# TurakhiaLab/DIPPER

Hardware: AMD Instinct MI355X
Metric: tips/sec FASTA->Newick at N=30000 (higher is better)
Workload: dtype f64

## Files before the change

### dipper_amd/csrc/njp.hip

```cpp
#include "njp_args.hpp"

#include <algorithm>
#include <chrono>
#include <cstdio>
#include <cstdlib>
#include <functional>
#include <numeric>
#include <string>
#include <type_traits>

namespace dpr {

static int64_t njp_big_p()
{
    static const int64_t v = std::getenv("DPR_NJ_BIG_P") ? std::atoll(std::getenv("DPR_NJ_BIG_P")) : 40000;
    return v;
}
static bool njp_post2_on()
{
    static const bool on = !(std::getenv("DPR_NJP_POST2") && std::atoi(std::getenv("DPR_NJP_POST2")) == 0);
    return on;
}
static int njp_tg(int64_t P) { return P < njp_big_p() ? 64 : 256; }
constexpr int kBigNS = 4;
static int njp_ns(int64_t P) { return P < njp_big_p() ? 1 : kBigNS; }
__host__ __device__ inline int64_t njp_strips_of_rows(int64_t g0, int64_t tg, int64_t P)
{
    const int64_t G16 = (P + 16 - 1) / 16;
    const int64_t glast = (g0 + tg < G16 ? g0 + tg : G16) - 1;
    if (glast < 0) return 0;
    int64_t c = glast / 32 + 1;
    const int64_t cp = (P - 2) / 512 + 1;
    return P >= 2 ? (c < cp ? c : cp) : 0;
}

int njp_unit_owner(int64_t strip, int64_t group, int64_t P, int world)
{
    const int64_t G16 = (P + kUR - 1) / kUR;
    if (strip < 0 || group < 0 || group >= G16 || group < 32 * strip || strip * kTileCols >= P - 1 || world < 1) return -1;
    int64_t t = 0;
    const int64_t tg = njp_tg(P), ns = njp_ns(P);
    if (ns == 1) {
        for (int64_t c = 0; c < strip; ++c) t += (G16 - 32 * c + tg - 1) / tg;
        t += (group - 32 * strip) / tg;
    } else {
        const int64_t k = group / tg;
        for (int64_t kk = 0; kk < k; ++kk) t += (njp_strips_of_rows(kk * tg, tg, P) + ns - 1) / ns;
        t += strip / ns;
    }
    return (int)(t % world);
}

__device__ __forceinline__ void njp_note_range(unsigned long long* mm, double lo, double hi)
{
    if (lo < 0.0) {
        const double cur = dec_f64(mm[0]);
        if (cur >= 0.0 || lo < 2.0 * cur) atomicMin(&mm[0], (unsigned long long)enc_f64(lo));
    }
    if (hi > 0.0) {
        const double cur = dec_f64(mm[1]);
        if (hi > 2.0 * cur) atomicMax(&mm[1], (unsigned long long)enc_f64(hi));
    }
}

__global__ __launch_bounds__(kThreads) void njp_permute_kernel(const double* __restrict__ A, int64_t lda,
                                                               double* __restrict__ B, int64_t ldb,
                                                               const int32_t* __restrict__ perm, int64_t P)
{
    const int xcd = (int)(blockIdx.x & 7u), chunk = (int)(blockIdx.x >> 3), nchunk = (int)(gridDim.x >> 3);
    for (int64_t a = (int64_t)blockIdx.y * 8 + xcd; a < P; a += (int64_t)gridDim.y * 8) {
        const double* row = A + (int64_t)perm[a] * lda;
        for (int64_t b = (int64_t)chunk * kThreads + threadIdx.x; b < P; b += (int64_t)nchunk * kThreads)
            B[a * ldb + b] = row[perm[b]];
    }
}

static void njp_launch_permute(const double* A, int64_t lda, double* B, int64_t ldb, const int32_t* perm, int64_t n, hipStream_t s)
{
    int64_t chunks = (n + 1023) / 1024;
    chunks = chunks < 1 ? 1 : (chunks > 64 ? 64 : chunks);
    const int64_t gy = (n + 7) / 8;
    dim3 grid((unsigned)(8 * chunks), (unsigned)(gy < 32768 ? gy : 32768));
    hipLaunchKernelGGL(njp_permute_kernel, grid, dim3(kThreads), 0, s, A, lda, B, ldb, perm, n);
}

__global__ __launch_bounds__(kThreads) void njp_range_kernel(const double* __restrict__ A, int64_t lda, int64_t n, unsigned long long* __restrict__ mm)
{
    __shared__ double slo[kThreads / 64], shi[kThreads / 64];
    double lo = __builtin_inf(), hi = 0.0;
    for (int64_t a = blockIdx.x; a < n; a += gridDim.x) {
        const double* row = A + a * lda;
        for (int64_t b = threadIdx.x; b < n; b += kThreads) {
            const double v = row[b];
            lo = fmin(lo, v); hi = fmax(hi, fabs(v));
        }
    }
    lo = wave_fmin(lo); hi = wave_fmax(hi);
    if ((threadIdx.x & 63) == 0) { slo[threadIdx.x >> 6] = lo; shi[threadIdx.x >> 6] = hi; }
    __syncthreads();
    if (threadIdx.x == 0) {
        for (int w = 1; w < kThreads / 64; ++w) { lo = fmin(lo, slo[w]); hi = fmax(hi, shi[w]); }
        atomicMin(&mm[0], (unsigned long long)enc_f64(lo));
        atomicMax(&mm[1], (unsigned long long)enc_f64(hi));
    }
}

__global__ __launch_bounds__(kThreads) void njp_init_vectors_kernel(const double* __restrict__ U_src,
                                                                    const int32_t* __restrict__ perm,
                                                                    const int32_t* __restrict__ slot_src,
                                                                    int64_t P, int64_t n, double* __restrict__ U,
                                                                    double* __restrict__ Ur, uint64_t* __restrict__ KA,
                                                                    uint64_t* __restrict__ KB,
                                                                    int32_t* __restrict__ slot_of_pos,
                                                                    int32_t* __restrict__ pos_of_slot)
{
    const int64_t p = (int64_t)blockIdx.x * kThreads + threadIdx.x;
    if (p >= P) return;
    const int32_t src = perm[p];
    const int32_t slot = slot_src ? slot_src[src] : src;
    const double u = U_src[src];
    U[p] = u;
    Ur[p] = u / (double)(n - 2);
    KA[p] = nj_key_a_dev(slot, n);
    KB[p] = nj_key_b(slot);
    slot_of_pos[p] = slot;
    pos_of_slot[slot] = (int32_t)p;
}

__global__ void njp_fill_u64_kernel(uint64_t* __restrict__ a, int64_t cnt, uint64_t v)
{
    for (int64_t i = (int64_t)blockIdx.x * blockDim.x + threadIdx.x; i < cnt; i += (int64_t)gridDim.x * blockDim.x) a[i] = v;
}

__global__ __launch_bounds__(kThreads) void njp_list_all_kernel(NjpArgs a)
{
    const int tid = threadIdx.x;
    const int64_t it = a.st->it;
    if (a.st->status != 0) return;
    const int tb = a.sh_rank + (int)blockIdx.x * a.sh_world;
    const int cb0 = a.blk_cb[tb];
    const int64_t g = (int64_t)a.blk_g0[tb] + tid;
    const int64_t G16 = (a.P + kUR - 1) / kUR;
    const int tg = a.tg;
    int64_t send = njp_strips_of_rows((int64_t)a.blk_g0[tb], tg, a.P);
    if (a.ns == 1) send = cb0 + 1;
    else if (send > cb0 + a.ns) send = cb0 + a.ns;
    const int lane = tid & 63;
    for (int cb = cb0; cb < (int)send; ++cb) {
        const bool keep = g < G16 && g >= 32 * (int64_t)cb && tid < tg;
        const unsigned long long mask = __ballot(keep);
        unsigned long long base = 0;
        if (lane == 0 && mask) base = atomicAdd(&a.cnt[it % 3], (unsigned long long)__popcll(mask));
        base = __shfl(base, 0, 64);
        if (keep) a.list[base + __popcll(mask & ((1ull << lane) - 1ull))] = (int32_t)((0xFu << 28) | ((uint32_t)cb << 18) | (uint32_t)g);
    }
}

template <bool kRS>
__global__ __launch_bounds__(kThreads) void njp_scan_kernel(NjState* h_st, const int32_t* h_list, const unsigned long long* h_cnt,
                                                            const double* h_xpart, int h_nrl, NjpArgs a)
{
    __shared__ double sq[kThreads / 64], sd[kThreads / 64];
    __shared__ uint64_t sk[kThreads / 64], sp[kThreads / 64];
    __shared__ double stree[kThreads];
    __shared__ unsigned int s_last;

    const int tid = threadIdx.x;
    const int64_t it = h_st->it, limit = h_st->it_limit, N = h_st->N;
    const int nrl = h_nrl;
    const bool unit_block = (int)blockIdx.x >= nrl;
    const int ub = (int)blockIdx.x - nrl;
    const int32_t first = unit_block ? h_list[ub] : 0;
    const double xp0 = unit_block ? 0.0 : h_xpart[tid];
    const unsigned long long cl0 = h_cnt[0], cl1 = h_cnt[1], cl2 = h_cnt[2];
    const int64_t j0 = (int64_t)blockIdx.x * kTileCols + 2 * tid;
    v2d dv0, dv1, uv; ulonglong2 kav, kbv;
    dv0.x = dv0.y = 0.0; dv1 = dv0; uv = dv0; kav = make_ulonglong2(0ull, 0ull); kbv = kav;
    if (!unit_block) {
        dv0 = *reinterpret_cast<const v2d*>(a.R + j0);
        dv1 = *reinterpret_cast<const v2d*>(a.R + a.vstride + j0);
        uv = *reinterpret_cast<const v2d*>(a.Ur + j0);
        kav = *reinterpret_cast<const ulonglong2*>(a.KA + j0); kbv = *reinterpret_cast<const ulonglong2*>(a.KB + j0);
    }
    const int32_t pn0 = h_st->pnew[0], pn1 = h_st->pnew[1];
    const int64_t pz = (int64_t)((it & 1) ? pn1 : pn0);
    if (blockIdx.x == 0 && tid == 0) h_st->itb = it;
    if (it >= limit || h_st->status != 0) return;
    NJP_STAMP(0, 0, true);
    const int64_t P = a.P;
    double bq = 10000.0, bd = 0.0;
    uint64_t bk = ~0ull, bp = 0;
    NjRecord* rec_out;

    if (!unit_block) {
        const int r = (int)blockIdx.x;
        rec_out = a.partials + a.urecs + r;
        if (pz < 0) {
            if (tid == 0) { NjRecord rec; rec.q = 10000.0; rec.key = ~0ull; rec.d = 0.0; rec.pad = 0ull; *rec_out = rec; }
            if (kRS) {
                if (r == 0 && tid == 0) njr_store_record(a.partials + a.rec_off - 1, 10000.0, ~0ull, it == a.rs_fault_it ? 1.0e-3 : 0.0, a.rs_seq_base + (unsigned long long)(it + 1));
                njr_scan_publish(a, it, &s_last);
            }
            return;
        }
        const int64_t n = N - it;
        const int64_t nchunk = (n + 1 + kThreads - 1) / kThreads;
        double acc = tid < nchunk ? xp0 : 0.0;
        for (int64_t c = tid + kThreads; c < nchunk; c += kThreads) acc += a.xpart[c];
        const v2d dv = ((it + 1) & 1) ? dv1 : dv0;
        const uint64_t kax = a.KA[pz], kbx = a.KB[pz];
        NJP_STAMP(0, 1, true);
        double ux = block_tree256_lane0(acc, stree);
        if (tid == 0) stree[0] = ux;
        __syncthreads();
        ux = stree[0];
        NJP_STAMP(0, 2, false);
        const double urx = ux / (double)(n - 2);
        if (r == 0 && tid == 0) a.U[(it & 1) * a.vstride + pz] = ux;
        if (kRS && r == 0 && tid == 0)
            njr_store_record(a.partials + a.rec_off - 1, 10000.0, ~0ull, it == a.rs_fault_it ? ux * 0.5 + 1.0e-3 : ux, a.rs_seq_base + (unsigned long long)(it + 1));
        if (j0 < P && njp_owns<kRS>(a, pz)) *reinterpret_cast<v2d*>(a.D + njp_lrow<kRS>(a, pz) * a.ld + j0) = dv;
#pragma unroll
        for (int k = 0; k < 2; ++k) {
            const double d = k ? dv.y : dv.x, uj = k ? uv.y : uv.x;
            const uint64_t kaj = k ? kav.y : kav.x, kbj = k ? kbv.y : kbv.x;
            const uint64_t pj = (uint64_t)(j0 + k);
            best_update4(bq, bk, bp, bd, (d - urx) - uj, kax | kbj, (uint64_t)pz | (pj << 32), d);
            best_update4(bq, bk, bp, bd, (d - uj) - urx, kaj | kbx, pj | ((uint64_t)pz << 32), d);
        }
        wave_best4(bq, bk, bp, bd);
    } else {
        rec_out = a.partials + a.rec_off + ub;
        const int m3 = (int)(it % 3);
        const int64_t cnt = (int64_t)(m3 == 0 ? cl0 : m3 == 1 ? cl1 : cl2);
        if ((int64_t)ub >= cnt) {
            if (a.all_defined && tid == 0) {
                if (kRS) njr_store_record(rec_out, 10000.0, ~0ull, 0.0, 0ull);
                else { NjRecord rec; rec.q = 10000.0; rec.key = ~0ull; rec.d = 0.0; rec.pad = 0ull; *rec_out = rec; }
            }
            if (kRS) njr_scan_publish(a, it, &s_last);
            return;
        }
        const int64_t G16 = (P + kUR - 1) / kUR;
        int64_t scanned = 0;
        const int wv = tid >> 6;
        for (int64_t e = ub; e < cnt; e += a.ugrid, ++scanned) {
            const uint32_t code = (uint32_t)__builtin_amdgcn_readfirstlane(e == (int64_t)ub ? first : a.list[e]);
            if (!((code >> (28 + wv)) & 1u)) continue;
            const int cb = (int)((code >> 18) & 1023u);
            const int64_t g_s = (int64_t)(code & 0x3FFFFu);
            const int64_t c0 = (int64_t)cb * kTileCols, a0 = g_s * kUR;
            const int64_t b0 = c0 + 2 * tid, b1 = b0 + 1;
            const v2d ubv = *reinterpret_cast<const v2d*>(a.Ur + b0);
            const ulonglong2 kav = *reinterpret_cast<const ulonglong2*>(a.KA + b0), kbv = *reinterpret_cast<const ulonglong2*>(a.KB + b0);
            const double ub0 = ubv.x, ub1 = ubv.y;
            const uint64_t ka0 = kav.x, ka1 = kav.y, kb0 = kbv.x, kb1 = kbv.y;
            const v2d* basep = reinterpret_cast<const v2d*>(a.D + njp_lrow<kRS>(a, a0) * a.ld + c0) + tid;
            const int64_t ld2 = a.ld >> 1;
            const bool diag = a0 < c0 + kTileCols;
            const bool live0 = ub0 == ub0, live1 = ub1 == ub1;
            v2d v[kUR];
#pragma unroll
            for (int u8 = 0; u8 < kUR; ++u8) v[u8] = __builtin_nontemporal_load(basep + (int64_t)u8 * ld2);
            const double ua_l = a.Ur[a0 + (tid & 15)];
            const uint64_t kaa_l = a.KA[a0 + (tid & 15)], kba_l = a.KB[a0 + (tid & 15)];
            double ua[kUR];
#pragma unroll
            for (int u8 = 0; u8 < kUR; ++u8) ua[u8] = readlane_f64(ua_l, u8);
            NJP_STAMP(0, 1, true);
            if (diag) {
                const int ib0 = (int)b0, ia0 = (int)a0;
#pragma unroll
                for (int u8 = 0; u8 < kUR; ++u8) {
                    const int ar = ia0 + u8;
                    v[u8].x = (ib0 < ar) ? v[u8].x : __builtin_nan("");
                    v[u8].y = (ib0 + 1 < ar) ? v[u8].y : __builtin_nan("");
                }
            }
            double lm = __builtin_inf(), m0 = __builtin_inf(), m1 = __builtin_inf();
            double rowq[kUR];
#pragma unroll
            for (int u8 = 0; u8 < kUR; ++u8) {
                const double d0 = v[u8].x, d1 = v[u8].y;
                const double rn = ua[u8] == ua[u8] ? 0.0 : __builtin_nan("");
                m0 = fmin(m0, d0 + rn);
                m1 = fmin(m1, d1 + rn);
                const double q0 = (d0 - ua[u8]) - ub0;
                const double q1 = (d0 - ub0) - ua[u8];
                const double q2 = (d1 - ua[u8]) - ub1;
                const double q3 = (d1 - ub1) - ua[u8];
                rowq[u8] = fmin(fmin(q0, q1), fmin(q2, q3));
                lm = fmin(lm, rowq[u8]);
            }
            double m = fmin(fmin(live0 ? m0 : __builtin_nan(""), live1 ? m1 : __builtin_nan("")), __builtin_inf());
            const double wm = wave_fmin(lm);
            NJP_STAMP(0, 2, false);
            if (wm <= bq) {
                if (wm < bq) { bq = wm; bk = ~0ull; }
                if (a.dbg != nullptr && (it == a.dbg_it || a.dbg_it == -2) && (tid & 63) == 0) atomicAdd(&a.dbg[(a.dbg_it == -2 ? 0 : (int)blockIdx.x) * 8 + 6], 1ull);
#pragma unroll
                for (int u8 = 0; u8 < kUR; ++u8) {
                    if (__builtin_amdgcn_ballot_w64(rowq[u8] == wm) != 0ull) {
                        if (a.dbg != nullptr && (it == a.dbg_it || a.dbg_it == -2) && (tid & 63) == 0) atomicAdd(&a.dbg[(a.dbg_it == -2 ? 0 : (int)blockIdx.x) * 8 + 5], 1ull);
                        double d0 = v[u8].x, d1 = v[u8].y;
                        asm volatile("" : "+v"(d0), "+v"(d1));
                        const bool e0 = (d0 - ua[u8]) - ub0 == wm, e1 = (d0 - ub0) - ua[u8] == wm;
                        const bool e2 = (d1 - ua[u8]) - ub1 == wm, e3 = (d1 - ub1) - ua[u8] == wm;
                        const uint64_t pa = (uint64_t)(a0 + u8);
                        const uint64_t kaa = readlane_u64(kaa_l, u8), kba = readlane_u64(kba_l, u8);
                        const uint64_t k0 = kaa | kb0, k1 = ka0 | kba, k2 = kaa | kb1, k3 = ka1 | kba;
                        if (e0 & (k0 < bk)) { bk = k0; bp = pa | ((uint64_t)b0 << 32); bd = d0; }
                        if (e1 & (k1 < bk)) { bk = k1; bp = (uint64_t)b0 | (pa << 32); bd = d0; }
                        if (e2 & (k2 < bk)) { bk = k2; bp = pa | ((uint64_t)b1 << 32); bd = d1; }
                        if (e3 & (k3 < bk)) { bk = k3; bp = (uint64_t)b1 | (pa << 32); bd = d1; }
                    }
                }
            }
            NJP_STAMP(0, 7, false);
            m = wave_fmin(m);
            if ((tid & 63) == 0) a.umin[((int64_t)cb * G16 + g_s) * 4 + wv] = enc_f64(m);
        }
        {
            const uint64_t wk = wave_umin64(bk);
            if (wk != ~0ull) {
                const unsigned long long own = __builtin_amdgcn_ballot_w64(bk == wk);
                const int src = __builtin_amdgcn_readfirstlane((int)__builtin_ctzll(own));
                bp = readlane_u64(bp, src);
                bd = readlane_f64(bd, src);
            }
            bk = wk;
        }
        if (tid == 0) {
            if (ub == 0) atomicAdd(&a.st->units_scanned, (unsigned long long)cnt);
        }
    }
    NJP_STAMP(0, 3, false);
    if ((tid & 63) == 0) { sq[tid >> 6] = bq; sk[tid >> 6] = bk; sp[tid >> 6] = bp; sd[tid >> 6] = bd; }
    __syncthreads();
    if (tid == 0) {
#pragma unroll
        for (int w = 1; w < kThreads / 64; ++w) best_update4(bq, bk, bp, bd, sq[w], sk[w], sp[w], sd[w]);
        if (kRS && unit_block) njr_store_record(rec_out, bq, bk, bd, bp);
        else {
            NjRecord rec;
            rec.q = bq; rec.key = bk; rec.d = bd; rec.pad = bp;
            *rec_out = rec;
        }
    }
    if (kRS) njr_scan_publish(a, it, &s_last);
    NJP_STAMP(0, 4, true);
}

template <bool kRS>
__global__ __launch_bounds__(kThreads) void njp_finish_kernel(NjpArgs a)
{
    __shared__ double stree[kThreads];
    const int tid = threadIdx.x;
    const int64_t it = a.st->it, N = a.st->N;
    const int64_t pz = (int64_t)a.st->pnew[it & 1];
    if (a.st->status != 0 || pz < 0) return;
    const int64_t n = N - it;
    const int64_t nchunk = (n + 1 + kThreads - 1) / kThreads;
    double acc = 0.0;
    for (int64_t c = tid; c < nchunk; c += kThreads) acc += a.xpart[c];
    const double* __restrict__ Rz = a.R + ((it + 1) & 1) * a.vstride;
    const int64_t j0 = (int64_t)blockIdx.x * kTileCols + 2 * tid;
    const v2d dv = *reinterpret_cast<const v2d*>(Rz + j0);
    const double ux = block_tree256_lane0(acc, stree);
    if (blockIdx.x == 0 && tid == 0) a.U[(it & 1) * a.vstride + pz] = ux;
    if (j0 < a.P && njp_owns<kRS>(a, pz)) *reinterpret_cast<v2d*>(a.D + njp_lrow<kRS>(a, pz) * a.ld + j0) = dv;
}

#ifndef DPR_NJP_BIG_WAVES
#define DPR_NJP_BIG_WAVES 1
#endif
template <int kTG, int kNS, bool kRS>
__global__ __launch_bounds__(kThreads, (kNS > 1 ? DPR_NJP_BIG_WAVES : 1)) void njp_post_kernel(NjState* h_st, const NjRecord* h_partials, const unsigned long long* h_cnt, const int32_t* h_blk_cb,
                                                                                              const int32_t* h_blk_g0, const int32_t* h_pos_of_slot, int h_ntest, int h_nupd, NjpArgs a)
{
    __shared__ double s[kThreads];
    __shared__ double sq[kThreads / 64], sdd[kThreads / 64];
    __shared__ uint64_t sk[kThreads / 64], spp[kThreads / 64];
    __shared__ double sseed[kThreads / 64];
    const int tid = threadIdx.x;
    const int bx = (int)blockIdx.x;
    const bool test_block = bx < h_ntest;
    const int tbi = bx, ubi = bx - h_ntest;
    const int tb = test_block ? a.sh_rank + tbi * a.sh_world : 0;
    const int64_t it = h_st->itb;
    const int64_t limit = h_st->it_limit, N = h_st->N;
    const int32_t pn0 = h_st->pnew[0], pn1 = h_st->pnew[1];
    const int64_t pz = (int64_t)((it & 1) ? pn1 : pn0);
    const int nrec_all = a.urecs + a.nrb;
    NjRecord r0; r0.q = 10000.0; r0.key = ~0ull; r0.d = 0; r0.pad = 0;
    constexpr int kMine = 5;
    NjRecord mine[kMine] = { r0, r0, r0, r0, r0 };
#pragma unroll
    for (int k = 0; k < kMine; ++k) {
        const int idx = tid + k * kThreads;
        if (idx < nrec_all) mine[k] = h_partials[idx];
    }
    const int nseed_rows = a.nrb < kThreads / 2 ? a.nrb : kThreads / 2;
    const int nseed_units = kThreads - nseed_rows;
    const int64_t sstride = a.all_defined && a.urecs >= 2 * nseed_units ? a.urecs / nseed_units : 1;
    const bool seed_is_unit = tid < nseed_units;
    NjRecord cand = r0;
    if (test_block) {
        if (!seed_is_unit) cand = h_partials[a.urecs + (tid - nseed_units)];
        else if ((int64_t)tid * sstride < a.urecs) cand = h_partials[(int64_t)tid * sstride];
    }
    const unsigned long long cl0 = h_cnt[0], cl1 = h_cnt[1], cl2 = h_cnt[2];
    const int m3 = (int)(it % 3);
    const unsigned long long cnt_raw = a.all_defined ? (unsigned long long)a.urecs : (m3 == 0 ? cl0 : m3 == 1 ? cl1 : cl2);
    const int64_t uvalid = (int64_t)(cnt_raw < (unsigned long long)a.urecs ? cnt_raw : (unsigned long long)a.urecs);
    const double* __restrict__ Uc = a.U + (it & 1) * a.vstride;
    double* __restrict__ Un = a.U + ((it + 1) & 1) * a.vstride;
    const int64_t P = a.P;
    const int64_t G16 = (P + kUR - 1) / kUR;
    const int64_t pclamp = (P + 1) & ~(int64_t)1;
    const int64_t i = (int64_t)ubi * kThreads + tid;
    int64_t p = -1;
    double up = 0.0;
    struct ColData { v2d ucol, dxc, dyc, rzc; ulonglong2 um0, um1; };
    int cb0 = 0, nsb = 0;
    int64_t g = 0, rbase = 0;
    bool have_g = false;
    constexpr int kRC = kTG * kUR / kTileCols;
    v2d urow[kRC];
    ColData cd[kNS];
#pragma unroll
    for (int k = 0; k < kNS; ++k) {
        cd[k].ucol.x = 0.0; cd[k].ucol.y = 0.0; cd[k].dxc = cd[k].ucol; cd[k].dyc = cd[k].ucol; cd[k].rzc = cd[k].ucol;
        cd[k].um0 = make_ulonglong2(0ull, 0ull); cd[k].um1 = cd[k].um0;
    }
    auto load_a = [&](int cb, ColData& c) {
        const int64_t pc0 = (int64_t)cb * kTileCols + 2 * tid;
        c.ucol = *reinterpret_cast<const v2d*>(Uc + pc0);
        if (have_g && g >= 32 * (int64_t)cb) {
            const unsigned long long* up = a.umin + ((int64_t)cb * G16 + g) * 4;
            c.um0 = *reinterpret_cast<const ulonglong2*>(up); c.um1 = *reinterpret_cast<const ulonglong2*>(up + 2);
        }
    };
    if (test_block) {
        cb0 = h_blk_cb[tb];
        g = (int64_t)h_blk_g0[tb] + tid;
        have_g = g < G16 && tid < kTG;
        rbase = (int64_t)h_blk_g0[tb] * kUR;
        if (kNS == 1) nsb = 1;
        else {
            const int64_t send = njp_strips_of_rows((int64_t)h_blk_g0[tb], kTG, P);
            nsb = (int)(send - cb0 < kNS ? send - cb0 : kNS);
        }
#pragma unroll
        for (int k = 0; k < kNS; ++k)
            if (k < nsb) load_a(cb0 + k, cd[k]);
#pragma unroll
        for (int c = 0; c < kRC; ++c) {
            const int64_t pp = rbase + c * kTileCols + 2 * tid;
            urow[c] = *reinterpret_cast<const v2d*>(Uc + (pp < P ? pp : pclamp));
        }
    } else {
        p = (int64_t)h_pos_of_slot[i];
    }
#pragma unroll
    for (int k = 0; k < kMine; ++k) {
        const int idx = tid + k * kThreads;
        if (idx >= uvalid && idx < a.urecs) mine[k] = r0;
    }
    if (!test_block) up = (i < N && p >= 0) ? Uc[p] : 0.0;
    if (h_st->status != 0 || it >= limit) return;
    const int64_t n = N - it;
    if (n < 3) return;
    if (!test_block && (!a.do_update || (int64_t)ubi * kThreads >= n)) return;
    if (test_block && !a.do_tests) return;
    NJP_STAMP(1, 0, false);
    NJP_STAMP(1, 1, true);

    double bq = 10000.0, d = 0.0; uint64_t bk = ~0ull, bp = 0;
    const int nmine = (nrec_all + kThreads - 1) / kThreads;
#pragma unroll
    for (int k = 0; k < kMine; ++k)
        if (k < nmine) best_update4(bq, bk, bp, d, mine[k].q, mine[k].key, mine[k].pad, mine[k].d);
    for (int64_t idx = tid + kMine * kThreads; idx < nrec_all; idx += kThreads)
        if (idx < uvalid || idx >= a.urecs) best_update4(bq, bk, bp, d, a.partials[idx].q, a.partials[idx].key, a.partials[idx].pad, a.partials[idx].d);
    wave_best4(bq, bk, bp, d);
    if ((tid & 63) == 0) { sq[tid >> 6] = bq; sk[tid >> 6] = bk; spp[tid >> 6] = bp; sdd[tid >> 6] = d; }
    __syncthreads();
    bq = sq[0]; bk = sk[0]; bp = spp[0]; d = sdd[0];
#pragma unroll
    for (int w = 1; w < kThreads / 64; ++w) best_update4(bq, bk, bp, d, sq[w], sk[w], spp[w], sdd[w]);

    NJP_STAMP(1, 2, false);
    const int64_t last = n - 1;
    if (bk == ~0ull || !(bq < 10000.0)) {
        if (!test_block && i == last) a.st->status = 1;
        return;
    }
    const int64_t ki = (int64_t)(bk & 0xFFFFFFull), kj = (int64_t)((bk >> 24) & 0xFFFFFFull);
    const int64_t pi = (int64_t)(bp & 0xffffffffull), pj = (int64_t)(bp >> 32);
    const int64_t x = ki < kj ? ki : kj, y = ki < kj ? kj : ki;
    const int64_t px = ki < kj ? pi : pj, py = ki < kj ? pj : pi;
    const int64_t n1 = n - 1;
    const double r1 = (double)(n1 - 2);
    const double* __restrict__ rowx = kRS ? a.rs_rows : a.D + px * a.ld;
    const double* __restrict__ rowy = kRS ? a.rs_rows + a.rs_slice : a.D + py * a.ld;
    auto RX = [&](int64_t pp_) -> const double* { return kRS ? rowx + njp_xoff(a, pp_) : rowx + pp_; };
    auto RY = [&](int64_t pp_) -> const double* { return kRS ? rowy + njp_xoff(a, pp_) : rowy + pp_; };
    if (kRS && a.rs_plan == kNjrMailbox) {
        __shared__ int s_fail;
        if (tid == 0) s_fail = 0;
        __syncthreads();
        if (tid < a.rs_world) {
            const unsigned long long* f = njr_win_rowflag(a.rs_win[a.rs_rank], a.rs_lay, tid);
            const unsigned long long want = a.rs_seq_base + (unsigned long long)(it + 1), t0 = wall_clock64();
            while (njr_ld_sys(f) != want) {
                if (wall_clock64() - t0 > a.rs_poll_ticks) { s_fail = 1; break; }
                __builtin_amdgcn_s_sleep(1);
            }
        }
        __syncthreads();
        if (s_fail) {
            if (!test_block && i == last) a.st->status = 3;
            return;
        }
    }

    if (!test_block) {
        double* __restrict__ Rw = a.R + (it & 1) * a.vstride;
        double val = 0.0;
        if (i < n) {
            if (i == last) {
                const double r = (double)(n - 2);
                double blX = (d + Uc[px] / r - Uc[py] / r) * 0.5;
                double blY = d - blX;
                if (blX < 0) { blY += blX; blX = 0; }
                if (blY < 0) { blX += blY; blY = 0; }
                a.log_x[it] = (int32_t)x; a.log_y[it] = (int32_t)y; a.log_bx[it] = blX; a.log_by[it] = blY;
                a.st->x = (int32_t)x; a.st->y = (int32_t)y; a.st->d = d; a.st->q = bq;
                a.st->n = n1; a.st->it = it + 1;
                a.st->pnew[(it + 1) & 1] = (int32_t)px;
                a.U[(it & 1) * a.vstride + py] = __builtin_nan("");
                a.st->cnt_list[(it + 2) % 3] = 0ull;
                for (int v = 0; v < a.cnt_ranks; ++v) a.cnt_all[4 * v + (it + 2) % 3] = 0ull;
            }
            int64_t new_slot = i;
            if (i != x && i != y) {
                const double dxi = *RX(p), dyi = *RY(p);
                val = nj_val(dxi, dyi, d);
                const double u = nj_unew(up, dxi, dyi, val);
                Un[p] = u;
                a.Ur[p] = u / r1;
                Rw[p] = val;
                if (kRS) { if (njp_owns<true>(a, p)) __hip_atomic_store(a.D + njp_lrow<true>(a, p) * a.ld + px, val, __ATOMIC_RELAXED, __HIP_MEMORY_SCOPE_AGENT); }
                else __hip_atomic_store(a.D + p * a.ld + px, val, __ATOMIC_RELAXED, __HIP_MEMORY_SCOPE_AGENT);
                if (i == last) {
                    new_slot = y;
                    a.slot_of_pos[p] = (int32_t)y;
                    a.pos_of_slot[y] = (int32_t)p;
                }
            } else if (i == y) {
                a.Ur[py] = __builtin_nan("");
                Un[py] = __builtin_nan("");
                a.slot_of_pos[py] = -1;
                Rw[py] = 0.0;
                new_slot = -1;
            } else {
                a.Ur[px] = __builtin_nan("");
                Rw[px] = 0.0;
            }
            if (new_slot >= 0) { a.KA[p] = nj_key_a_dev(new_slot, n1); a.KB[p] = nj_key_b(new_slot); }
        }
        NJP_STAMP(1, 3, false);
        const double cs = block_tree256_lane0(val, s);
        if (tid == 0) a.xpart[ubi] = cs;
        NJP_STAMP(1, 6, true);
        return;
    }

    const double NINF = -__builtin_inf(), PINF = __builtin_inf();
    const bool fold = pz >= 0 && pz != px && pz != py;
    const double* __restrict__ Rz = a.R + ((it + 1) & 1) * a.vstride;
    const int64_t gz = fold ? pz / kUR : -1;
    const bool gz_here = fold && gz >= (int64_t)a.blk_g0[tb] && gz < (int64_t)a.blk_g0[tb] + kTG;
    const int wpz = fold ? (int)((pz % kTileCols) / (kTileCols / 4)) : -1;
    auto load_b = [&](int cb, ColData& c) {
        const int64_t pc0 = (int64_t)cb * kTileCols + 2 * tid;
        c.dxc = *reinterpret_cast<const v2d*>(RX(pc0));
        c.dyc = *reinterpret_cast<const v2d*>(RY(pc0));
        c.rzc.x = PINF; c.rzc.y = PINF;
        if (gz_here) c.rzc = *reinterpret_cast<const v2d*>(Rz + pc0);
    };
    constexpr bool kPreRz = kRC <= 4;
    const bool pz_block = fold && pz / kTileCols >= cb0 && pz / kTileCols < cb0 + nsb;
    v2d dxr[kRC], dyr[kRC], rzr[kPreRz ? kRC : 1];
#pragma unroll
    for (int c = 0; c < kRC; ++c) {
        const int64_t pp = rbase + c * kTileCols + 2 * tid;
        const int64_t po = pp < P ? pp : pclamp;
        dxr[c] = *reinterpret_cast<const v2d*>(RX(po));
        dyr[c] = *reinterpret_cast<const v2d*>(RY(po));
        if (kPreRz) {
            rzr[c].x = 0.0; rzr[c].y = 0.0;
            if (pz_block) rzr[c] = *reinterpret_cast<const v2d*>(Rz + po);
        }
    }
#pragma unroll
    for (int k = 0; k < kNS; ++k)
        if (k < nsb) load_b(cb0 + k, cd[k]);
    double qc = PINF;
    if (seed_is_unit && (int64_t)tid * sstride >= uvalid) cand.key = ~0ull;
    if (cand.key != ~0ull) {
        const int64_t ci = (int64_t)(cand.pad & 0xffffffffull), cj = (int64_t)(cand.pad >> 32);
        if (ci < P && cj < P && ci != px && cj != px && ci != py && cj != py) {
            const double uia = Uc[ci], uib = Uc[cj];
            const double xa = *RX(ci), ya = *RY(ci), xb = *RX(cj), yb = *RY(cj);
            const double ua = nj_unew(uia, xa, ya, nj_val(xa, ya, d)) / r1;
            const double ub = nj_unew(uib, xb, yb, nj_val(xb, yb, d)) / r1;
            const double qk = fmin((cand.d - ua) - ub, (cand.d - ub) - ua);
            qc = qk == qk ? qk : qc;
        }
    }
    NJP_STAMP(1, 3, true);
    __shared__ double s_un[kTG * (kUR + 1)];
    __shared__ double scm2[2][kThreads / 64], snew2[2][kThreads / 64];
    const int lxp = (int)(px - rbase), lyp = (int)(py - rbase), lzp = (int)((fold ? pz : -1) - rbase);
#pragma unroll
    for (int c = 0; c < kRC; ++c) {
        const int lp = c * kTileCols + 2 * tid;
        const double u0 = urow[c].x, u1 = urow[c].y;
        const bool live0 = (u0 == u0) & (lp != lxp) & (lp != lyp);
        const bool live1 = (u1 == u1) & (lp + 1 != lxp) & (lp + 1 != lyp);
        const double n0 = nj_unew(u0, dxr[c].x, dyr[c].x, nj_val(dxr[c].x, dyr[c].x, d));
        const double n1v = nj_unew(u1, dxr[c].y, dyr[c].y, nj_val(dxr[c].y, dyr[c].y, d));
        const int li = lp + (lp >> 4);
        s_un[li] = live0 ? n0 : NINF;
        s_un[li + 1] = live1 ? n1v : NINF;
    }
    qc = wave_fmin(qc);
    if ((tid & 63) == 0) sseed[tid >> 6] = qc;
    double bound = PINF, rmax = NINF;
    const int tg = tid < kTG ? tid : 0;
    const int lane = tid & 63;
#pragma unroll
    for (int sidx = 0; sidx < kNS; ++sidx) {
        if (sidx >= nsb) break;
        const int cb = cb0 + sidx, par = sidx & 1;
        const ColData& cur = cd[sidx];
        const int64_t pc0 = (int64_t)cb * kTileCols + 2 * tid;
        const bool pz_strip = fold && pz / kTileCols == cb;
        const bool have = have_g && g >= 32 * (int64_t)cb;
        unsigned long long* up4 = a.umin + ((int64_t)cb * G16 + (have ? g : 0)) * 4;
        double u4[4] = { PINF, PINF, PINF, PINF };
        if (have) { u4[0] = dec_f64(cur.um0.x); u4[1] = dec_f64(cur.um0.y); u4[2] = dec_f64(cur.um1.x); u4[3] = dec_f64(cur.um1.y); }
        double cm_part = NINF, colmin = PINF;
#pragma unroll
        for (int k = 0; k < 2; ++k) {
            const int64_t pp = pc0 + k;
            const double uo = k ? cur.ucol.y : cur.ucol.x;
            const double dx = k ? cur.dxc.y : cur.dxc.x, dy = k ? cur.dyc.y : cur.dyc.x;
            const double rz = k ? cur.rzc.y : cur.rzc.x;
            const bool live = (uo == uo) & (pp != px) & (pp != py) & (pp < P);
            const double un = nj_unew(uo, dx, dy, nj_val(dx, dy, d));
            cm_part = live ? fmax(cm_part, un) : cm_part;
            colmin = (live & (pp < pz)) ? fmin(colmin, rz) : colmin;
        }
        cm_part = wave_fmax(cm_part) / r1;
        if (gz_here) colmin = wave_fmin(colmin);
        if (lane == 0) { scm2[par][tid >> 6] = cm_part; snew2[par][tid >> 6] = colmin; }
        __syncthreads();
        NJP_STAMP(1, 4, false);
        if (sidx == 0) {
            bound = fmin(fmin(sseed[0], sseed[1]), fmin(sseed[2], sseed[3]));
#pragma unroll
            for (int k = 0; k < kUR; ++k) rmax = fmax(rmax, s_un[17 * tg + k]);
            rmax = rmax / r1;
        }
        double newminA = PINF;
        if (pz_strip) {
            __syncthreads();
#pragma unroll
            for (int c = 0; c < kRC; ++c) {
                const int lp = c * kTileCols + 2 * tid;
                const int64_t pp = rbase + lp;
                const v2d rz = kPreRz ? rzr[kPreRz ? c : 0] : *reinterpret_cast<const v2d*>(Rz + (pp < P ? pp : pclamp));
                const double u0 = urow[c].x, u1 = urow[c].y;
                const bool live0 = (u0 == u0) & (lp != lxp) & (lp != lyp) & (lp > lzp);
                const bool live1 = (u1 == u1) & (lp + 1 != lxp) & (lp + 1 != lyp) & (lp + 1 > lzp);
                const int li = lp + (lp >> 4);
                s_un[li] = live0 ? rz.x : PINF;
                s_un[li + 1] = live1 ? rz.y : PINF;
            }
            __syncthreads();
#pragma unroll
            for (int k = 0; k < kUR; ++k) newminA = fmin(newminA, s_un[17 * tg + k]);
        }
        int submask = 0;
        if (have) {
#pragma unroll
            for (int w = 0; w < 4; ++w) {
                const double cmw = scm2[par][w];
                double nm = (gz_here && g == gz) ? snew2[par][w] : PINF;
                if (pz_strip && w == wpz) nm = fmin(nm, newminA);
                if (nm < u4[w]) {
                    u4[w] = nm;
                    up4[w] = enc_f64(nm);
                }
                const double lb = fmin((u4[w] - rmax) - cmw, (u4[w] - cmw) - rmax);
                if ((cmw > NINF) && (lb <= bound)) submask |= 1 << w;
            }
        }
        const bool keep = have && (rmax > NINF) && submask != 0;
        const unsigned long long mask = __ballot(keep);
        unsigned long long base = 0;
        if (lane == 0 && mask) base = atomicAdd(&a.cnt[(it + 1) % 3], (unsigned long long)__popcll(mask));
        base = __shfl(base, 0, 64);
        if (a.dbg != nullptr && a.dbg_it == -2 && mask) {
            int subs = keep ? __popc(submask) : 0;
            for (int off = 32; off > 0; off >>= 1) subs += __shfl_xor(subs, off, 64);
            if (lane == 0 && it < 32768) {
                atomicMax(&a.dbg[32768 + it], ((unsigned long long)__popcll(mask) << 32) | (unsigned long long)subs);
                atomicAdd(&a.dbg[7], (unsigned long long)subs);
            }
        }
        NJP_STAMP(1, 5, true);
        if (keep) a.list[base + __popcll(mask & ((1ull << lane) - 1ull))] = (int32_t)(((uint32_t)submask << 28) | ((uint32_t)cb << 18) | (uint32_t)g);
    }
    NJP_STAMP(1, 6, true);
}

struct Post2Hdr { unsigned long long min_enc, maxabs_enc; };

__global__ __launch_bounds__(kThreads) void njp_t2_init_kernel(const double* __restrict__ Uc, int64_t P, double* __restrict__ rmaxU,
                                                               double* __restrict__ cmaxU)
{
    const int tid = threadIdx.x;
    const int64_t p0 = (int64_t)blockIdx.x * kTileCols + 2 * tid;
    const v2d uc = *reinterpret_cast<const v2d*>(Uc + p0);
    const double NINF = -__builtin_inf();
    const double m2 = fmax(((uc.x == uc.x) & (p0 < P)) ? uc.x : NINF, ((uc.y == uc.y) & (p0 + 1 < P)) ? uc.y : NINF);
    double gm = m2;
    gm = fmax(gm, __shfl_xor(gm, 1, 64)); gm = fmax(gm, __shfl_xor(gm, 2, 64)); gm = fmax(gm, __shfl_xor(gm, 4, 64));
    const double cm = wave_fmax(m2);
    if ((tid & 7) == 0) rmaxU[p0 >> 4] = gm;
    if ((tid & 63) == 0) cmaxU[4 * blockIdx.x + (tid >> 6)] = cm;
}

template <int kNS>
__global__ __launch_bounds__(kThreads) void njp_post2_kernel(NjState* h_st, const NjRecord* h_partials, const unsigned long long* h_cnt, const int32_t* h_blk_cb,
                                                         const int32_t* h_blk_g0, const int32_t* h_pos_of_slot, int h_ntest, int h_nupd, NjpArgs a)
{
    constexpr int kTG = 256;
    __shared__ double s[kThreads];
    __shared__ double sq[kThreads / 64], sdd[kThreads / 64];
    __shared__ uint64_t sk[kThreads / 64], spp[kThreads / 64];
    __shared__ double sseed[kThreads / 64], srC[kThreads / 64], scm[kNS * 4], s_colmin[kNS * 4];
    const int tid = threadIdx.x;
    const int lane = tid & 63;
    const int bx = (int)blockIdx.x;
    const bool trole = bx < h_ntest;
    const int tb = a.sh_rank + bx * a.sh_world;
    const int umb = bx - h_ntest;
    Post2Hdr* hdr = reinterpret_cast<Post2Hdr*>(a.t2_hdr);
    const double NINF = -__builtin_inf(), PINF = __builtin_inf();

    const int64_t it = h_st->itb;
    const int64_t limit = h_st->it_limit, N = h_st->N;
    const int32_t pn0 = h_st->pnew[0], pn1 = h_st->pnew[1];
    const int64_t pz = (int64_t)((it & 1) ? pn1 : pn0);
    const int64_t P = a.P;
    const int64_t G16 = (P + kUR - 1) / kUR;
    const int nrec_all = a.urecs + a.nrb;
    NjRecord r0; r0.q = 10000.0; r0.key = ~0ull; r0.d = 0; r0.pad = 0;
    constexpr int kMine = 5;
    NjRecord mine[kMine] = { r0, r0, r0, r0, r0 };
#pragma unroll
    for (int k = 0; k < kMine; ++k) {
        const int idx = tid + k * kThreads;
        if (idx < nrec_all) mine[k] = h_partials[idx];
    }
    const int nseed_rows = a.nrb < kThreads / 2 ? a.nrb : kThreads / 2;
    const int nseed_units = kThreads - nseed_rows;
    const int64_t sstride = a.all_defined && a.urecs >= 2 * nseed_units ? a.urecs / nseed_units : 1;
    const bool seed_is_unit = tid < nseed_units;
    NjRecord cand = r0;
    int cb0 = 0;
    int64_t g0 = 0;
    const int64_t i = (int64_t)umb * (2 * kThreads) + tid;
    const int64_t p0 = (int64_t)umb * kTileCols + 2 * tid;
    const bool m_part = !trole && umb < a.nrb && a.do_update;
    const bool u_slots = !trole && (int64_t)umb * (2 * kThreads) < N;
    int64_t p = -1, pb = -1;
    int2 sl = make_int2(-1, -1);
    if (trole) {
        if (!seed_is_unit) cand = h_partials[a.urecs + (tid - nseed_units)];
        else if ((int64_t)tid * sstride < a.urecs) cand = h_partials[(int64_t)tid * sstride];
        cb0 = h_blk_cb[tb];
        g0 = (int64_t)h_blk_g0[tb];
    } else {
        if (u_slots) { p = (int64_t)h_pos_of_slot[i]; pb = (int64_t)h_pos_of_slot[i + kThreads]; }
        if (m_part) sl = *reinterpret_cast<const int2*>(a.slot_of_pos + p0);
    }
    const int par = (int)(it & 1);
    const double* __restrict__ Uc = a.U + (it & 1) * a.vstride;
    double* __restrict__ Un = a.U + ((it + 1) & 1) * a.vstride;
    const unsigned long long cl0 = h_cnt[0], cl1 = h_cnt[1], cl2 = h_cnt[2];
    const int m3 = (int)(it % 3);
    const unsigned long long cnt_raw = a.all_defined ? (unsigned long long)a.urecs : (m3 == 0 ? cl0 : m3 == 1 ? cl1 : cl2);
    const int64_t uvalid = (int64_t)(cnt_raw < (unsigned long long)a.urecs ? cnt_raw : (unsigned long long)a.urecs);
    const double emin = dec_f64(hdr->min_enc), eabs = dec_f64(hdr->maxabs_enc);
    v2d uc; uc.x = 0.0; uc.y = 0.0;
    const int64_t g = g0 + tid;
    const bool have_g = trole && g < G16;
    int nsb = 0;
    double uz = NINF;
    double sUa = 0.0, sUb = 0.0;
    int64_t ci = -1, cj = -1;
    if (m_part) uc = *reinterpret_cast<const v2d*>(Uc + p0);
    if (trole) {
        const int64_t send = njp_strips_of_rows(g0, kTG, P);
        nsb = (int)(send - cb0 < kNS ? send - cb0 : kNS);
        if (pz >= 0) uz = Uc[pz];
        if (seed_is_unit && (int64_t)tid * sstride >= uvalid) cand.key = ~0ull;
        if (cand.key != ~0ull) {
            ci = (int64_t)(cand.pad & 0xffffffffull); cj = (int64_t)(cand.pad >> 32);
            if (!(ci < P && cj < P)) ci = -1;
        }
    }
#pragma unroll
    for (int k = 0; k < kMine; ++k) {
        const int idx = tid + k * kThreads;
        if (idx >= uvalid && idx < a.urecs) mine[k] = r0;
    }
    NJP_STAMP(1, 0, false);
    NJP_STAMP(1, 1, true);
    if (h_st->status != 0 || it >= limit) return;
    const int64_t n = N - it;
    if (n < 3) return;
    const bool u_part = u_slots && a.do_update && (int64_t)umb * (2 * kThreads) < n;
    if (trole ? !a.do_tests : (!u_part && !m_part)) return;

    double bq = 10000.0, d = 0.0; uint64_t bk = ~0ull, bp = 0;
    const int nmine = (nrec_all + kThreads - 1) / kThreads;
#pragma unroll
    for (int k = 0; k < kMine; ++k)
        if (k < nmine) best_update4(bq, bk, bp, d, mine[k].q, mine[k].key, mine[k].pad, mine[k].d);
    for (int64_t idx = tid + kMine * kThreads; idx < nrec_all; idx += kThreads)
        if (idx < uvalid || idx >= a.urecs) best_update4(bq, bk, bp, d, a.partials[idx].q, a.partials[idx].key, a.partials[idx].pad, a.partials[idx].d);
    wave_best4(bq, bk, bp, d);
    if (lane == 0) { sq[tid >> 6] = bq; sk[tid >> 6] = bk; spp[tid >> 6] = bp; sdd[tid >> 6] = d; }
    __syncthreads();
    bq = sq[0]; bk = sk[0]; bp = spp[0]; d = sdd[0];
#pragma unroll
    for (int w = 1; w < kThreads / 64; ++w) best_update4(bq, bk, bp, d, sq[w], sk[w], spp[w], sdd[w]);

    NJP_STAMP(1, 2, false);
    const int64_t last = n - 1;
    if (bk == ~0ull || !(bq < 10000.0)) {
        if (u_part && (i == last || i + kThreads == last)) a.st->status = 1;
        return;
    }
    const int64_t ki = (int64_t)(bk & 0xFFFFFFull), kj = (int64_t)((bk >> 24) & 0xFFFFFFull);
    const int64_t pi = (int64_t)(bp & 0xffffffffull), pj = (int64_t)(bp >> 32);
    const int64_t x = ki < kj ? ki : kj, y = ki < kj ? kj : ki;
    const int64_t px = ki < kj ? pi : pj, py = ki < kj ? pj : pi;
    const int64_t n1 = n - 1;
    const double r1 = (double)(n1 - 2);
    const double* __restrict__ rowx = a.D + px * a.ld;
    const double* __restrict__ rowy = a.D + py * a.ld;
    const int64_t GS = 32 * ((P + kTileCols - 1) / kTileCols + 2), SS4 = 4 * ((P + kTileCols - 1) / kTileCols + 2);

    if (!trole) {
        double gx[2] = { 0.0, 0.0 }, gy[2] = { 0.0, 0.0 };
        v2d dx, dy; dx.x = dx.y = dy.x = dy.y = 0.0;
        if (u_part) {
#pragma unroll
            for (int h = 0; h < 2; ++h) {
                const int64_t ii = i + h * kThreads, pp = h ? pb : p;
                if (ii < n && ii != x && ii != y) { gx[h] = rowx[pp]; gy[h] = rowy[pp]; }
            }
        }
        if (m_part) { dx = *reinterpret_cast<const v2d*>(rowx + p0); dy = *reinterpret_cast<const v2d*>(rowy + p0); }
        if (m_part) {
            const bool live0 = (uc.x == uc.x) & (p0 != px) & (p0 != py) & (p0 < P);
            const bool live1 = (uc.y == uc.y) & (p0 + 1 != px) & (p0 + 1 != py) & (p0 + 1 < P);
            const double v0 = nj_val(dx.x, dy.x, d), v1 = nj_val(dx.y, dy.y, d);
            const double un0 = nj_unew(uc.x, dx.x, dy.x, v0);
            const double un1 = nj_unew(uc.y, dx.y, dy.y, v1);
            NJP_STAMP(2, 4, false);
            if (a.do_update) {
                double* __restrict__ Rw = a.R + (it & 1) * a.vstride;
#pragma unroll
                for (int k = 0; k < 2; ++k) {
                    const int64_t pp = p0 + k;
                    const int slot = k ? sl.y : sl.x;
                    const double v = k ? v1 : v0, u = k ? un1 : un0;
                    if (pp >= P) continue;
                    if (pp == px) {
                        a.Ur[px] = __builtin_nan("");
                        Rw[px] = 0.0;
                        a.KA[px] = nj_key_a_dev(x, n1); a.KB[px] = nj_key_b(x);
                    } else if (pp == py) {
                        a.Ur[py] = __builtin_nan("");
                        Un[py] = __builtin_nan("");
                        Rw[py] = 0.0;
                    } else if (slot >= 0) {
                        Un[pp] = u;
                        a.Ur[pp] = u / r1;
                        Rw[pp] = v;
                        __hip_atomic_store(a.D + pp * a.ld + px, v, __ATOMIC_RELAXED, __HIP_MEMORY_SCOPE_AGENT);
                        const int64_t new_slot = slot == (int)last ? y : (int64_t)slot;
                        a.KA[pp] = nj_key_a_dev(new_slot, n1); a.KB[pp] = nj_key_b(new_slot);
                    }
                }
            }
            NJP_STAMP(2, 5, false);
            const double m2 = fmax(live0 ? un0 : NINF, live1 ? un1 : NINF);
            double gm = m2;
            gm = fmax(gm, __shfl_xor(gm, 1, 64)); gm = fmax(gm, __shfl_xor(gm, 2, 64)); gm = fmax(gm, __shfl_xor(gm, 4, 64));
            const double cm = wave_fmax(m2);
            const int64_t gidx = p0 >> 4;
            const int wq = 1 - par;
            if ((tid & 7) == 0) a.t2_rmax[wq * GS + gidx] = gm;
            if (lane == 0) a.t2_cmax[wq * SS4 + 4 * umb + (tid >> 6)] = cm;
            const double c2 = fmin((live0 & (p0 < px)) ? v0 : PINF, (live1 & (p0 + 1 < px)) ? v1 : PINF);
            double r2 = fmin((live0 & (p0 > px)) ? v0 : PINF, (live1 & (p0 + 1 > px)) ? v1 : PINF);
            r2 = fmin(r2, __shfl_xor(r2, 1, 64)); r2 = fmin(r2, __shfl_xor(r2, 2, 64)); r2 = fmin(r2, __shfl_xor(r2, 4, 64));
            const double cz = wave_fmin(c2);
            if ((tid & 7) == 0) a.t2_rowmin[wq * GS + gidx] = r2;
            if (lane == 0) a.t2_colmin[wq * SS4 + 4 * umb + (tid >> 6)] = cz;
            double vmin = fmin(live0 ? v0 : PINF, live1 ? v1 : PINF);
            double vabs = fmax(live0 ? fabs(v0) : 0.0, live1 ? fabs(v1) : 0.0);
            vmin = wave_fmin(vmin); vabs = wave_fmax(vabs);
            if (lane == 0) njp_note_range(&hdr->min_enc, vmin, vabs);
        }
        NJP_STAMP(1, 3, true);
        if (u_part) {
            double val2[2] = { 0.0, 0.0 };
#pragma unroll
            for (int h = 0; h < 2; ++h) {
                const int64_t ii = i + h * kThreads;
                const int64_t pp = h ? pb : p;
                if (ii >= n) continue;
                if (ii == last) {
                    const double r = (double)(n - 2);
                    double blX = (d + Uc[px] / r - Uc[py] / r) * 0.5;
                    double blY = d - blX;
                    if (blX < 0) { blY += blX; blX = 0; }
                    if (blY < 0) { blX += blY; blY = 0; }
                    a.log_x[it] = (int32_t)x; a.log_y[it] = (int32_t)y; a.log_bx[it] = blX; a.log_by[it] = blY;
                    a.st->x = (int32_t)x; a.st->y = (int32_t)y; a.st->d = d; a.st->q = bq;
                    a.st->n = n1; a.st->it = it + 1;
                    a.st->pnew[(it + 1) & 1] = (int32_t)px;
                    a.U[(it & 1) * a.vstride + py] = __builtin_nan("");
                    a.st->cnt_list[(it + 2) % 3] = 0ull;
                    for (int v = 0; v < a.cnt_ranks; ++v) a.cnt_all[4 * v + (it + 2) % 3] = 0ull;
                }
                if (ii != x && ii != y) {
                    val2[h] = nj_val(gx[h], gy[h], d);
                    if (ii == last) {
                        a.slot_of_pos[pp] = (int32_t)y;
                        a.pos_of_slot[y] = (int32_t)pp;
                    }
                } else if (ii == y) {
                    a.slot_of_pos[py] = -1;
                }
            }
            const double cs0 = block_tree256_lane0(val2[0], s);
            if (tid == 0) a.xpart[2 * umb] = cs0;
            if ((int64_t)(2 * umb + 1) * kThreads < n) {
                __syncthreads();
                const double cs1 = block_tree256_lane0(val2[1], s);
                if (tid == 0) a.xpart[2 * umb + 1] = cs1;
            }
        }
        NJP_STAMP(1, 6, true);
        if (a.dbg != nullptr && it == a.dbg_it && tid == 0 && bx < 2048) a.dbg[(2048 + bx) * 8 + 7] = 1ull;
        return;
    }

    const double rmaxU = have_g ? a.t2_rmax[par * GS + g] : NINF;
    double cmU = NINF;
    if (tid < 4 * kNS && (tid >> 2) < nsb) cmU = a.t2_cmax[par * SS4 + 4 * (cb0 + (tid >> 2)) + (tid & 3)];
    const double cmin = a.t2_cmin[tb];
    double qc = PINF;
    {
        const bool live = ci >= 0 && ci != px && cj != px && ci != py && cj != py;
        const double oq = live ? cand.q : PINF;
        constexpr int sgm = 0;
        bool lead = live;
        if (sgm != 3) {
            double gmin = oq;
            gmin = fmin(gmin, dpp_f64<kDppXor1>(gmin));
            gmin = fmin(gmin, dpp_f64<kDppXor2>(gmin));
            gmin = fmin(gmin, dpp_f64<kDppHalfMirror>(gmin));
            if (sgm != 2) gmin = fmin(gmin, dpp_f64<kDppMirror>(gmin));
            if (sgm == 1) gmin = fmin(fmin(readlane_f64(gmin, 0), readlane_f64(gmin, 16)), fmin(readlane_f64(gmin, 32), readlane_f64(gmin, 48)));
            const int sgl = sgm == 1 ? 64 : sgm == 2 ? 8 : 16;
            const unsigned long long hit = __builtin_amdgcn_ballot_w64(live & (oq == gmin));
            const int gbase = lane & ~(sgl - 1);
            const unsigned long long mine_g = (hit >> gbase) & (sgl == 64 ? ~0ull : ((1ull << sgl) - 1ull));
            lead = live && mine_g != 0ull && (lane - gbase) == (int)__builtin_ctzll(mine_g);
        }
        if (lead) {
            sUa = Uc[ci]; sUb = Uc[cj];
            const double xa = rowx[ci], ya = rowy[ci], xb = rowx[cj], yb = rowy[cj];
            const double ua = nj_unew(sUa, xa, ya, nj_val(xa, ya, d)) / r1;
            const double ub = nj_unew(sUb, xb, yb, nj_val(xb, yb, d)) / r1;
            const double qk = fmin((cand.d - ua) - ub, (cand.d - ub) - ua);
            qc = qk == qk ? qk : qc;
        }
    }
    ulonglong2 um0[kNS], um1[kNS];
#pragma unroll
    for (int k = 0; k < kNS; ++k) { um0[k] = make_ulonglong2(0ull, 0ull); um1[k] = um0[k]; }
    if (kNS == 1 && nsb > 0 && have_g && g >= 32 * (int64_t)cb0) {
        const unsigned long long* up = a.umin + ((int64_t)cb0 * G16 + g) * 4;
        um0[0] = *reinterpret_cast<const ulonglong2*>(up); um1[0] = *reinterpret_cast<const ulonglong2*>(up + 2);
    }
    qc = wave_fmin(qc);
    if (lane == 0) sseed[tid >> 6] = qc;
    NJP_STAMP(1, 3, true);
    const double slack = emin >= 0.0 ? 0.0 : (3.0 * -emin) * (1.0 + 0x1p-30) + eabs * 0x1p-47;
    const bool zlive = pz >= 0 && pz != px && pz != py;
    uz = (uz == uz) ? uz : PINF;
    const int64_t gz = zlive ? pz / kUR : -1;
    const int64_t sz = zlive ? pz / (kTileCols / 4) : -1;
    double rU = rmaxU;
    if (have_g && g == gz) rU = fmax(rU, uz);
    const double rmax = (rU + slack) / r1;
    if (tid < 4 * kNS) {
        double cU = cmU;
        if (4 * (int64_t)(cb0 + (tid >> 2)) + (tid & 3) == sz) cU = fmax(cU, uz);
        scm[tid] = (cU + slack) / r1;
    }
    const bool fold = zlive;
    const bool gz_here = fold && gz >= g0 && gz < g0 + kTG;
    const int wpz = fold ? (int)((pz % kTileCols) / (kTileCols / 4)) : -1;
    const int64_t cbz = fold ? pz / kTileCols : -1;
    const bool pz_here = fold && cbz >= cb0 && cbz < cb0 + nsb;
    double rC = wave_fmax(rmax);
    if (lane == 0) srC[tid >> 6] = rC;
    __syncthreads();
    const double bound = fmin(fmin(sseed[0], sseed[1]), fmin(sseed[2], sseed[3]));
    double cm4[kNS][4];
#pragma unroll
    for (int k = 0; k < kNS; ++k)
#pragma unroll
        for (int w = 0; w < 4; ++w) cm4[k][w] = scm[4 * k + w];
    {
        rC = fmax(fmax(srC[0], srC[1]), fmax(srC[2], srC[3]));
        double cC = NINF;
#pragma unroll
        for (int k = 0; k < kNS; ++k)
#pragma unroll
            for (int w = 0; w < 4; ++w) cC = fmax(cC, cm4[k][w]);
        const double lbC = fmin((cmin - rC) - cC, (cmin - cC) - rC);
        if (!gz_here && !pz_here && !(lbC <= bound)) {
            NJP_STAMP(1, 6, false);
            if (a.dbg != nullptr && it == a.dbg_it && tid == 0) a.dbg[(2048 + bx) * 8 + 7] = 3ull;
            return;
        }
        NJP_STAMP(1, 4, false);
    }
    double colz = PINF;
    if (gz_here && tid < 4 * kNS && (tid >> 2) < nsb) colz = a.t2_colmin[par * SS4 + 4 * (cb0 + (tid >> 2)) + (tid & 3)];
    if (kNS > 1) {
#pragma unroll
        for (int k = 0; k < kNS; ++k) {
            if (k < nsb && have_g && g >= 32 * (int64_t)(cb0 + k)) {
                const unsigned long long* up = a.umin + ((int64_t)(cb0 + k) * G16 + g) * 4;
                um0[k] = *reinterpret_cast<const ulonglong2*>(up); um1[k] = *reinterpret_cast<const ulonglong2*>(up + 2);
            }
        }
    }
    NJP_STAMP(1, 5, true);
    if (gz_here) {
        if (tid < 4 * kNS) s_colmin[tid] = colz;
        __syncthreads();
    }
    double mymin = PINF;
    int sub[kNS];
#pragma unroll
    for (int sidx = 0; sidx < kNS; ++sidx) {
        sub[sidx] = 0;
        if (sidx >= nsb) continue;
        const int cb = cb0 + sidx;
        const bool pz_strip = fold && cbz == cb;
        const bool have = have_g && g >= 32 * (int64_t)cb;
        unsigned long long* up4 = a.umin + ((int64_t)cb * G16 + (have ? g : 0)) * 4;
        double u4[4] = { PINF, PINF, PINF, PINF };
        if (have) { u4[0] = dec_f64(um0[sidx].x); u4[1] = dec_f64(um0[sidx].y); u4[2] = dec_f64(um1[sidx].x); u4[3] = dec_f64(um1[sidx].y); }
        const double newminA = (pz_strip && have_g) ? a.t2_rowmin[par * GS + g] : PINF;
        int submask = 0;
        if (have) {
#pragma unroll
            for (int w = 0; w < 4; ++w) {
                const double cmw = cm4[sidx][w];
                double nm = (gz_here && g == gz) ? s_colmin[4 * sidx + w] : PINF;
                if (pz_strip && w == wpz) nm = fmin(nm, newminA);
                if (nm < u4[w]) {
                    u4[w] = nm;
                    up4[w] = enc_f64(nm);
                }
                mymin = fmin(mymin, u4[w]);
                const double lb = fmin((u4[w] - rmax) - cmw, (u4[w] - cmw) - rmax);
                if ((cmw > NINF) && (lb <= bound)) submask |= 1 << w;
            }
        }
        if (have && (rmax > NINF)) sub[sidx] = submask;
    }
    NJP_STAMP(2, 0, false);
    {
        unsigned long long masks[kNS];
        int total = 0;
#pragma unroll
        for (int sidx = 0; sidx < kNS; ++sidx) { masks[sidx] = __ballot(sub[sidx] != 0); total += __popcll(masks[sidx]); }
        if (total > 0) {
            unsigned long long base = 0;
            if (lane == 0) base = atomicAdd(&a.cnt[(it + 1) % 3], (unsigned long long)total);
            base = __shfl(base, 0, 64);
            NJP_STAMP(2, 1, false);
#pragma unroll
            for (int sidx = 0; sidx < kNS; ++sidx) {
                if (sub[sidx] != 0)
                    a.list[base + __popcll(masks[sidx] & ((1ull << lane) - 1ull))] =
                        (int32_t)(((uint32_t)sub[sidx] << 28) | ((uint32_t)(cb0 + sidx) << 18) | (uint32_t)g);
                base += (unsigned long long)__popcll(masks[sidx]);
            }
        }
    }
    NJP_STAMP(2, 2, false);
    mymin = wave_fmin(mymin);
    __syncthreads();
    if (lane == 0) srC[tid >> 6] = mymin;
    __syncthreads();
    NJP_STAMP(2, 3, false);
    if (tid == 0) a.t2_cmin[tb] = fmin(fmin(srC[0], srC[1]), fmin(srC[2], srC[3]));
    NJP_STAMP(1, 6, true);
    if (a.dbg != nullptr && it == a.dbg_it && tid == 0) a.dbg[(2048 + bx) * 8 + 7] = 4ull;
}

static int64_t round_up16(int64_t v) { return (v + 15) / 16 * 16; }
static unsigned long long* g_njp_dbg_last = nullptr;

[[maybe_unused]] static const void* const kNjpInstantiations[] = {
    (const void*)njp_scan_kernel<false>, (const void*)njp_post2_kernel<kBigNS>, (const void*)njp_post_kernel<64, 1, false>, (const void*)njp_post_kernel<256, kBigNS, false>,
    (const void*)njp_scan_kernel<true>, (const void*)njp_post_kernel<64, 1, true>, (const void*)njp_finish_kernel<true>, (const void*)njp_finish_kernel<false> };

int njp_launch_list_all(const NjpArgs& a, hipStream_t s)
{
    if (a.ntest > 0) hipLaunchKernelGGL(njp_list_all_kernel, dim3((unsigned)a.ntest), dim3(kThreads), 0, s, a);
    DPR_HIP(hipGetLastError());
    return DPR_OK;
}
int njp_launch_scan(const NjpArgs& a, hipStream_t s)
{
    const int nrl = a.do_rows ? a.nrb : 0;
    auto* kernel = a.rs_world > 0 ? njp_scan_kernel<true> : njp_scan_kernel<false>;
    hipLaunchKernelGGL(kernel, dim3((unsigned)(a.ugrid + nrl)), dim3(kThreads), 0, s, a.st, (const int32_t*)a.list, (const unsigned long long*)a.cnt,
                       (const double*)a.xpart, nrl, a);
    DPR_HIP(hipGetLastError());
    return DPR_OK;
}
int njp_launch_post(const NjpArgs& a0, int64_t N, bool post2, hipStream_t s)
{
    NjpArgs a = a0;
    unsigned ublocks = a.do_update ? (unsigned)((N + kThreads - 1) / kThreads) : 0u;
    if (post2 && a.do_update) {
        const unsigned u2 = (unsigned)((N + 2 * kThreads - 1) / (2 * kThreads));
        ublocks = u2 > (unsigned)a.nrb ? u2 : (unsigned)a.nrb;
    }
    a.nupd = (int)ublocks;
    if ((unsigned)a.ntest + ublocks == 0u) return DPR_OK;
    auto* kernel = a.rs_world > 0 ? njp_post_kernel<64, 1, true> : post2 ? njp_post2_kernel<kBigNS>
                 : a.tg == 64 ? njp_post_kernel<64, 1, false> : njp_post_kernel<256, kBigNS, false>;
    hipLaunchKernelGGL(kernel, dim3((unsigned)a.ntest + ublocks), dim3(kThreads), 0, s, a.st, (const NjRecord*)a.partials, (const unsigned long long*)a.cnt,
                       a.blk_cb, a.blk_g0, (const int32_t*)a.pos_of_slot, a.ntest, a.nupd, a);
    DPR_HIP(hipGetLastError());
    return DPR_OK;
}
int njp_launch_finish(const NjpArgs& a, hipStream_t s)
{
    auto* kernel = a.rs_world > 0 ? njp_finish_kernel<true> : njp_finish_kernel<false>;
    hipLaunchKernelGGL(kernel, dim3((unsigned)a.nrb), dim3(kThreads), 0, s, a);
    DPR_HIP(hipGetLastError());
    return DPR_OK;
}

static bool njp_use_post2(const NjPruned& q)
{
    const int ns = njp_ns(q.P);
    return njp_post2_on() && ns == kBigNS && (q.dbg == nullptr || q.dbg_it >= 0);
}

static size_t align256(size_t v) { return (v + 255) / 256 * 256; }
static int prep_blocks(int64_t P, int rs_world, int rs_rank, std::vector<int32_t>& hcb, std::vector<int32_t>& hg0)
{
    const int64_t G16 = (P + kUR - 1) / kUR;
    auto add = [&](int64_t c, int64_t g0) { hcb.push_back((int32_t)c); hg0.push_back((int32_t)g0); };
    if (rs_world > 1) {
        const int64_t gpc = kNjrChunk / kUR;
        for (int64_t c = 0; 32 * c < G16 && c * kTileCols < P - 1; ++c)
            for (int64_t g0 = (32 * c) / gpc * gpc; g0 < G16; g0 += gpc)
                if (njr_owner(g0 * kUR, rs_world) == rs_rank) add(c, g0);
    } else if (njp_ns(P) == 1) {
        for (int64_t c = 0; 32 * c < G16 && c * kTileCols < P - 1; ++c)
            for (int64_t g0 = 32 * c; g0 < G16; g0 += njp_tg(P)) add(c, g0);
    } else {
        for (int64_t g0 = 0; g0 < G16; g0 += njp_tg(P))
            for (int64_t c0 = 0; c0 < njp_strips_of_rows(g0, njp_tg(P), P); c0 += njp_ns(P)) add(c0, g0);
    }
    const int blocks = (int)hcb.size();
    if (blocks == 0) add(0, 0);
    return rs_world > 1 ? blocks : (int)hcb.size();
}
static int64_t vec_len(int64_t N) { return (N + kTileCols + 16 + 31) / 32 * 32; }

static int njp_carve(NjPruned* qp, char* slab, int64_t P, int64_t N, int local_ranks, hipStream_t s, size_t* total)
{
    NjPruned dry;
    NjPruned& q = slab ? *qp : dry;
    const size_t vec = (size_t)vec_len(N);
    const int64_t G16 = (P + kUR - 1) / kUR, S = (P + kTileCols - 1) / kTileCols + 1;
    size_t off = 0;
    hipError_t err = hipSuccess;
    auto take = [&](auto*& ptr, size_t count, int fill = -1) {
        using T = std::remove_reference_t<decltype(*ptr)>;
        if (slab) {
            ptr = reinterpret_cast<T*>(slab + off);
            if (fill >= 0 && err == hipSuccess) err = hipMemsetAsync(ptr, fill, count * sizeof(T), s);
        }
        off += align256(count * sizeof(T));
    };
    q.vstride = (int64_t)vec;
    take(q.U, 2 * vec, 0xff);
    take(q.R, 2 * vec, 0);
    take(q.Ur, vec, 0xff);
    take(q.KA, vec, 0);
    take(q.KB, vec, 0);
    take(q.slot_of_pos, vec, 0xff);
    take(q.pos_of_slot, vec, 0xff);
    take(q.perm, vec);
    q.nunits_alloc = S * G16 * 4;
    take(q.umin, (size_t)q.nunits_alloc);
    q.list_stride = unit_total(P) + kScanBlocks + 64;
    take(q.list, (size_t)(q.list_stride * local_ranks), 0);
    size_t nprep = 1;
    for (int64_t c = 0; 32 * c < G16 && c * kTileCols < P - 1; ++c) nprep += (size_t)((G16 - 32 * c + 31) / 32);
    take(q.blk_cb, nprep);
    take(q.blk_g0, nprep);
    take(q.cnt_all, (size_t)(4 * local_ranks), 0);
    take(q.t2_hdr, 256);
    take(q.t2_rmax, (size_t)(2 * 32 * (S + 1)));
    take(q.t2_rowmin, (size_t)(2 * 32 * (S + 1)));
    take(q.t2_cmax, (size_t)(2 * 4 * (S + 1)));
    take(q.t2_colmin, (size_t)(2 * 4 * (S + 1)));
    take(q.t2_cmin, nprep);
    *total = off;
    return err == hipSuccess ? DPR_OK : hip_fail(err, "hipMemsetAsync (epoch slab)");
}
static size_t matrix_bytes(int64_t N)
{
    const int64_t rows_alloc = (N + kRowBlock - 1) / kRowBlock * kRowBlock + 32;
    return (size_t)(rows_alloc * round_up16(N) + kTileCols + 16) * sizeof(double);
}

static int njp_local_ranks(const NjPruned& q) { return q.sh_world > 1 && q.sh_virtual ? q.sh_world : 1; }

static int njp_reserve_slabs(NjPruned& q, int64_t N, int local_ranks, bool with_matrix, hipStream_t s)
{
    size_t total = 0;
    if (int rc = njp_carve(nullptr, nullptr, N, N, local_ranks, nullptr, &total)) return rc;
    if (q.arena_slab[0] && (q.arena_D || !with_matrix) && q.arena_N == N && q.arena_ranks >= local_ranks && q.arena_slab_bytes >= total) return DPR_OK;
    void* old[] = { with_matrix ? q.arena_D : nullptr, q.arena_slab[0], q.arena_slab[1] };
    for (void* p : old)
        if (p) (void)hipFree(p);
    q.arena_slab[0] = q.arena_slab[1] = nullptr;
    if (with_matrix) {
        q.arena_D = nullptr;
        DPR_HIP(hipMalloc(&q.arena_D, matrix_bytes(N)));
        DPR_HIP(hipMemsetAsync(q.arena_D, 0, matrix_bytes(N), s));
    }
    for (int k = 0; k < 2; ++k) DPR_HIP(hipMalloc(&q.arena_slab[k], total));
    q.arena_slab_bytes = total; q.arena_N = N; q.arena_ranks = local_ranks;
    return DPR_OK;
}

int njp_arena(NjPruned& q, int64_t N, hipStream_t s) { return njp_reserve_slabs(q, N, njp_local_ranks(q), true, s); }

static int njp_alloc_epoch(NjPruned& q, int64_t P, int64_t N, double* Dbuf, char* slab, hipStream_t s, const void* hdr_from = nullptr,
                           int rs_world = 1, int rs_rank = 0)
{
    if (P >= (int64_t)kTileCols * 1024) { set_error("pruned NJ: the list encoding holds fewer than 524288 positions"); return DPR_ERR_ARG; }
    q.P = P;
    q.ld = round_up16(P);
    q.D = Dbuf;
    const int64_t rows_alloc = (P + kUR - 1) / kUR * kUR + kUR;
    if (rs_world <= 1)
        if (int rc = nj_fill_pads(q.D, q.ld, P, P, rows_alloc, kTileCols + 16, false, s)) return rc;
    std::vector<int32_t> hcb, hg0;
    q.nprep = prep_blocks(P, rs_world, rs_rank, hcb, hg0);
    q.utot = unit_total(P);
    size_t total = 0;
    if (int rc = njp_carve(&q, slab, P, N, njp_local_ranks(q), s, &total)) return rc;
    if (hdr_from != nullptr) {
        DPR_HIP(hipMemcpyAsync(q.t2_hdr, hdr_from, 16, hipMemcpyDeviceToDevice, s));
    } else {
        const unsigned long long h0[2] = { 0xFFF0000000000000ull , 0x8000000000000000ull  };
        DPR_HIP(hipMemcpyAsync(q.t2_hdr, h0, sizeof h0, hipMemcpyHostToDevice, s));
        DPR_HIP(hipStreamSynchronize(s));
    }
    DPR_HIP(hipMemcpyAsync(q.blk_cb, hcb.data(), sizeof(int32_t) * hcb.size(), hipMemcpyHostToDevice, s));
    DPR_HIP(hipMemcpyAsync(q.blk_g0, hg0.data(), sizeof(int32_t) * hg0.size(), hipMemcpyHostToDevice, s));
    DPR_HIP(hipStreamSynchronize(s));
    hipLaunchKernelGGL(njp_fill_u64_kernel, dim3(256), dim3(256), 0, s, (uint64_t*)q.umin, q.nunits_alloc,
                       enc_f64_host(-__builtin_inf()));
    hipLaunchKernelGGL(njp_fill_u64_kernel, dim3(16), dim3(256), 0, s, (uint64_t*)q.t2_cmin, (int64_t)q.nprep, 0xFFF0000000000000ull);
    DPR_HIP(hipGetLastError());
    q.fresh = true;
    return DPR_OK;
}

int njp_rs_epoch(NjPruned& q, int64_t P, int64_t N, double* Dbuf, int epoch_index, int rs_rank, int rs_world, const void* hdr_from, hipStream_t s)
{
    if (int rc = njp_reserve_slabs(q, N, 1, false, s)) return rc;
    if (q.graph) { (void)hipGraphExecDestroy(q.graph); q.graph = nullptr; }
    q.sh_world = 1; q.sh_rank = 0; q.sh_virtual = false;
    q.epoch_index = epoch_index;
    if (int rc = njp_alloc_epoch(q, P, N, Dbuf, q.arena_slab[epoch_index & 1], s, hdr_from, rs_world, rs_rank)) return rc;
    q.active = true;
    return DPR_OK;
}

int njp_epoch_order(const double* dU, const int32_t* slot_of_pos, int64_t P, int64_t n, std::vector<int32_t>& perm, bool stream_idle, hipStream_t s)
{
    std::vector<double> hU((size_t)P);
    if (stream_idle) {
        DPR_HIP(hipMemcpy(hU.data(), dU, sizeof(double) * (size_t)P, hipMemcpyDeviceToHost));
    } else {
        DPR_HIP(hipMemcpyAsync(hU.data(), dU, sizeof(double) * (size_t)P, hipMemcpyDeviceToHost, s));
        DPR_HIP(hipStreamSynchronize(s));
    }
    perm.clear();
    perm.reserve((size_t)n);
    if (slot_of_pos) {
        std::vector<int32_t> hslot((size_t)P);
        DPR_HIP(hipMemcpy(hslot.data(), slot_of_pos, sizeof(int32_t) * (size_t)P, hipMemcpyDeviceToHost));
        for (int64_t p = 0; p < P; ++p)
            if (hslot[(size_t)p] >= 0) perm.push_back((int32_t)p);
    } else {
        perm.resize((size_t)P);
        std::iota(perm.begin(), perm.end(), 0);
    }
    if ((int64_t)perm.size() != n) { set_error("pruned NJ epoch: live positions do not match the active size"); return DPR_ERR_STATE; }
    std::stable_sort(perm.begin(), perm.end(), [&](int32_t a, int32_t c) {
        const double ua = hU[(size_t)a], uc = hU[(size_t)c];
        if (ua != ua) return false;
        if (uc != uc) return true;
        return ua < uc;
    });
    return DPR_OK;
}
int njp_init_vectors(NjPruned& q, const double* U_src, const int32_t* slot_src, int64_t n, int64_t it, hipStream_t s)
{
    hipLaunchKernelGGL(njp_init_vectors_kernel, dim3((unsigned)((n + kThreads - 1) / kThreads)), dim3(kThreads), 0, s,
                       U_src, (const int32_t*)q.perm, slot_src, n, n, q.U + (it & 1) * q.vstride, q.Ur, q.KA, q.KB, q.slot_of_pos, q.pos_of_slot);
    DPR_HIP(hipGetLastError());
    return DPR_OK;
}
int njp_put_fresh_state(NjState* d_st, NjState& st, hipStream_t s)
{
    st.pnew[0] = -1; st.pnew[1] = -1;
    for (auto& c : st.cnt_list) c = 0ull;
    DPR_HIP(hipMemcpyAsync(d_st, &st, sizeof(NjState), hipMemcpyHostToDevice, s));
    return DPR_OK;
}
static int njp_find_range(NjPruned& q, const double* D, int64_t ld, int64_t n, hipStream_t s)
{
    q.range_known = njp_use_post2(q);
    if (!q.range_known) return DPR_OK;
    hipLaunchKernelGGL(njp_range_kernel, dim3(2048), dim3(kThreads), 0, s, D, ld, n, (unsigned long long*)q.t2_hdr);
    DPR_HIP(hipGetLastError());
    return DPR_OK;
}
void njp_plan_from_env(NjPruned& q)
{
    const char* e = std::getenv("DPR_NJP_GRID");
    const int g = e ? std::atoi(e) : 512;
    q.scan_grid = g < 1 ? 1 : (g > 1024 ? 1024 : g);
    if (const char* gi = std::getenv("DPR_NJ_GRAPH_ITERS")) { const int v = std::atoi(gi); if (v >= 1 && v <= 4096) q.graph_iters = v; }
}

int njp_build(NjBuffers& b, hipStream_t s)
{
    NjPruned& q = b.pr;
    njp_plan_from_env(q);
    if (const char* e = std::getenv("DPR_NJ_ADAPTIVE")) q.adaptive = std::atoi(e) != 0 ? 1 : 0;
    if (const char* e = std::getenv("DPR_NJ_STREAM_FRAC")) q.stream_frac = std::atof(e);
    q.stream_iterations = 0; q.stream_epochs = 0;
    if (const char* e = std::getenv("DPR_NJ_PHASES")) {
        q.dbg_it = std::atoll(e);
        if (!q.dbg) DPR_HIP(hipMalloc(&q.dbg, sizeof(unsigned long long) * 4 * 2048 * 8));
        DPR_HIP(hipMemsetAsync(q.dbg, 0, sizeof(unsigned long long) * 4 * 2048 * 8, s));
        g_njp_dbg_last = q.dbg;
    }
    const int64_t N = b.N;
    std::vector<int32_t> perm;
    if (int rc = njp_epoch_order(b.U, nullptr, N, N, perm, false, s)) return rc;
    if (int rc = njp_arena(q, N, s)) return rc;
    q.epoch_index = 0;
    if (int rc = njp_alloc_epoch(q, N, N, q.arena_D, q.arena_slab[0], s)) return rc;
    q.utot0 = q.utot;
    DPR_HIP(hipMemcpyAsync(q.perm, perm.data(), sizeof(int32_t) * (size_t)N, hipMemcpyHostToDevice, s));
    njp_launch_permute(b.D, b.ld, q.D, q.ld, q.perm, N, s);
    if (int rc = njp_find_range(q, b.D, b.ld, N, s)) return rc;
    if (int rc = njp_init_vectors(q, b.U, nullptr, N, 0, s)) return rc;
    DPR_HIP(hipStreamSynchronize(s));
    q.active = true;
    return DPR_OK;
}

static int njp_rebuild_epoch(NjBuffers& b, hipStream_t s, bool* rebuilt)
{
    NjPruned& q = b.pr;
    *rebuilt = false;
    const bool tlog = log_level("epoch") >= 3;
    auto tprev = std::chrono::steady_clock::now();
    auto lap = [&](const char* what) {
        if (!tlog) return;
        const auto t = std::chrono::steady_clock::now();
        std::fprintf(stderr, "[njp]   rebuild: %s %.3f ms\n", what, std::chrono::duration<double, std::milli>(t - tprev).count());
        tprev = t;
    };
    NjState st;
    DPR_HIP(hipMemcpy(&st, b.st, sizeof(NjState), hipMemcpyDeviceToHost));
    const int64_t n = st.n;
    if (st.status != 0 || n < 3) return DPR_OK;
    const double* Ucur = njp_current_u(q, st.it);
    std::vector<int32_t> perm;
    if (int rc = njp_epoch_order(Ucur, q.slot_of_pos, q.P, n, perm, true, s)) return rc;
    lap("state + vectors to the host, sort");
    if (q.graph) { (void)hipGraphExecDestroy(q.graph); q.graph = nullptr; }
    const NjPruned old = q;
    const int e = old.epoch_index + 1;
    q.epoch_index = e;
    if (int rc = njp_alloc_epoch(q, n, b.N, (e & 1) ? b.D : q.arena_D, q.arena_slab[e & 1], s, old.range_known ? old.t2_hdr : nullptr)) return rc;
    lap("njp_alloc_epoch");
    DPR_HIP(hipMemcpyAsync(q.perm, perm.data(), sizeof(int32_t) * (size_t)n, hipMemcpyHostToDevice, s));
    njp_launch_permute(old.D, old.ld, q.D, q.ld, q.perm, n, s);
    if (int rc = njp_init_vectors(q, Ucur, old.slot_of_pos, n, st.it, s)) return rc;
    if (int rc = njp_put_fresh_state(b.st, st, s)) return rc;
    lap("enqueue");
    DPR_HIP(hipStreamSynchronize(s));
    lap("device work");
    *rebuilt = true;
    return DPR_OK;
}

__global__ __launch_bounds__(kThreads) void njp_gather_u_kernel(const double* __restrict__ Ucur, const int32_t* __restrict__ pos_of_slot,
                                                                int64_t n, double* __restrict__ U)
{
    const int64_t s = (int64_t)blockIdx.x * kThreads + threadIdx.x;
    if (s < n) U[s] = Ucur[pos_of_slot[s]];
}

static int njp_to_slots(NjBuffers& b, hipStream_t s)
{
    NjPruned& q = b.pr;
    NjState st;
    DPR_HIP(hipMemcpy(&st, b.st, sizeof(NjState), hipMemcpyDeviceToHost));
    const int64_t n = st.n;
    if (st.status != 0 || n < 3) return DPR_OK;
    if (q.graph) { (void)hipGraphExecDestroy(q.graph); q.graph = nullptr; }
    if (q.D == b.D) std::swap(b.D, q.arena_D);
    njp_launch_permute((const double*)q.D, q.ld, b.D, b.ld, (const int32_t*)q.pos_of_slot, n, s);
    hipLaunchKernelGGL(njp_gather_u_kernel, dim3((unsigned)((n + kThreads - 1) / kThreads)), dim3(kThreads), 0, s,
                       njp_current_u(q, st.it), (const int32_t*)q.pos_of_slot, n, b.U);
    DPR_HIP(hipGetLastError());
    if (int rc = nj_prepare(b, s)) return rc;
    q.slots_mode = true;
    ++q.stream_epochs;
    return DPR_OK;
}

static int njp_from_slots(NjBuffers& b, hipStream_t s)
{
    NjPruned& q = b.pr;
    NjState st;
    DPR_HIP(hipStreamSynchronize(s));
    DPR_HIP(hipMemcpy(&st, b.st, sizeof(NjState), hipMemcpyDeviceToHost));
    const int64_t n = st.n;
    if (st.status != 0 || n < 3) return DPR_OK;
    std::vector<int32_t> perm;
    if (int rc = njp_epoch_order(b.U, nullptr, n, n, perm, true, s)) return rc;
    q.epoch_index = 0;
    if (int rc = njp_alloc_epoch(q, n, b.N, q.arena_D, q.arena_slab[0], s)) return rc;
    DPR_HIP(hipMemcpyAsync(q.perm, perm.data(), sizeof(int32_t) * (size_t)n, hipMemcpyHostToDevice, s));
    njp_launch_permute((const double*)b.D, b.ld, q.D, q.ld, (const int32_t*)q.perm, n, s);
    if (int rc = njp_find_range(q, b.D, b.ld, n, s)) return rc;
    if (int rc = njp_init_vectors(q, b.U, nullptr, n, st.it, s)) return rc;
    if (int rc = njp_put_fresh_state(b.st, st, s)) return rc;
    DPR_HIP(hipStreamSynchronize(s));
    q.slots_mode = false;
    return DPR_OK;
}

static int njp_run_slots(NjBuffers& b, int64_t it0, int64_t todo, hipStream_t s)
{
    const int64_t n0 = b.N - it0;
    for (int64_t k = 0; k < todo; ++k) {
        if (int rc = nj_launch_scan(b, false, n0 - k, it0 + k, s)) return rc;
        if (int rc = nj_launch_post(b, n0 - k, it0 + k, s)) return rc;
    }
    b.pr.stream_iterations += todo;
    return nj_launch_finish(b, n0 - todo, it0 + todo, s);
}

void njp_reset(NjPruned& q)
{
    if (q.graph) { (void)hipGraphExecDestroy(q.graph); q.graph = nullptr; }
    NjPruned fresh;
    fresh.arena_D = q.arena_D; fresh.arena_slab[0] = q.arena_slab[0]; fresh.arena_slab[1] = q.arena_slab[1];
    fresh.arena_slab_bytes = q.arena_slab_bytes; fresh.arena_N = q.arena_N; fresh.arena_ranks = q.arena_ranks;
    fresh.adaptive = q.adaptive;
    fresh.dbg = q.dbg;
    q = fresh;
}

void njp_free(NjPruned& q)
{
    njp_reset(q);
    if (q.dbg) { if (g_njp_dbg_last == q.dbg) g_njp_dbg_last = nullptr; (void)hipFree(q.dbg); q.dbg = nullptr; }
    void* ptrs[] = { q.arena_D, q.arena_slab[0], q.arena_slab[1] };
    for (void* p : ptrs)
        if (p) (void)hipFree(p);
    q = NjPruned();
}

static int njp_grid_rank(const NjPruned& q) { return q.sh_world > 1 ? (q.scan_grid / q.sh_world > 0 ? q.scan_grid / q.sh_world : 1) : q.scan_grid; }
static int njp_grid_total(const NjPruned& q) { return q.sh_world > 1 ? njp_grid_rank(q) * q.sh_world : q.scan_grid; }
static int njp_first_rank(const NjPruned& q) { return q.sh_world > 1 && !q.sh_virtual ? q.sh_rank : 0; }
static int njp_last_rank(const NjPruned& q) { return q.sh_world > 1 ? (q.sh_virtual ? q.sh_world : q.sh_rank + 1) : 1; }

static NjpArgs njp_args(NjBuffers& b, int v)
{
    NjPruned& q = b.pr;
    const bool sh = q.sh_world > 1;
    const int slot = sh && q.sh_virtual ? v : 0;
    NjpArgs a{};
    a.D = q.D; a.ld = q.ld; a.st = b.st;
    a.U = q.U; a.R = q.R; a.vstride = q.vstride;
    a.Ur = q.Ur; a.KA = q.KA; a.KB = q.KB; a.slot_of_pos = q.slot_of_pos; a.pos_of_slot = q.pos_of_slot;
    a.xpart = b.xpart; a.partials = b.partials; a.umin = (unsigned long long*)q.umin;
    a.P = q.P;
    a.blk_cb = q.blk_cb; a.blk_g0 = q.blk_g0;
    a.tg = njp_tg(q.P); a.ns = njp_ns(q.P); a.nupd = 0;
    a.ntest = sh ? (q.nprep - v + q.sh_world - 1) / q.sh_world : q.nprep;
    a.list = q.list + (int64_t)slot * q.list_stride;
    a.cnt = sh ? q.cnt_all + 4 * slot : b.st->cnt_list;
    a.ugrid = njp_grid_rank(q);
    a.urecs = njp_grid_total(q);
    a.nrb = (int)((q.P + kTileCols - 1) / kTileCols);
    a.rec_off = sh ? v * a.ugrid : 0;
    a.all_defined = sh ? 1 : 0;
    a.sh_rank = sh ? v : 0; a.sh_world = sh ? q.sh_world : 1;
    a.cnt_all = sh ? q.cnt_all : nullptr;
    a.cnt_ranks = sh ? (q.sh_virtual ? q.sh_world : 1) : 0;
    a.do_update = 1; a.do_tests = 1; a.do_rows = 1;
    a.log_x = b.log_x; a.log_y = b.log_y; a.log_bx = b.log_bx; a.log_by = b.log_by;
    a.dbg = q.dbg; a.dbg_it = q.dbg_it;
    a.t2_hdr = q.t2_hdr; a.t2_rmax = q.t2_rmax; a.t2_cmax = q.t2_cmax; a.t2_colmin = q.t2_colmin; a.t2_rowmin = q.t2_rowmin; a.t2_cmin = q.t2_cmin;
    return a;
}

static int njp_enqueue_iteration(NjBuffers& b, hipStream_t s, bool sample = false)
{
    NjPruned& q = b.pr;
    const bool post2 = njp_use_post2(q);
    if (q.sh_world <= 1) {
        const NjpArgs a = njp_args(b, 0);
        if (sample) { b.kt->nk = 3; njp_set_kernel_names(nullptr); }
        if (int rc = nj_timing_mark(b.kt, sample, s)) return rc;
        if (int rc = njp_launch_scan(a, s)) return rc;
        if (int rc = nj_timing_mark(b.kt, sample, s)) return rc;
        if (int rc = njp_launch_post(a, b.N, post2, s)) return rc;
        if (int rc = nj_timing_mark(b.kt, sample, s)) return rc;
        return nj_timing_mark(b.kt, sample, s);
    }
    const int v0 = njp_first_rank(q), v1 = njp_last_rank(q);
    for (int v = v0; v < v1; ++v) {
        NjpArgs a = njp_args(b, v);
        a.do_rows = v == v0 ? 1 : 0;
        if (int rc = njp_launch_scan(a, s)) return rc;
    }
    if (!q.sh_virtual) {
        if (!q.gather) { set_error("njp: unit-sharded mode without a gather callback"); return DPR_ERR_STATE; }
        if (int rc = q.gather(q.gather_ctx, b.partials, sizeof(NjRecord) * (size_t)njp_grid_rank(q), s)) return rc;
    }
    for (int v = v0; v < v1; ++v) {
        NjpArgs a = njp_args(b, v);
        a.do_update = v == v0 ? 1 : 0;
        if (int rc = njp_launch_post(a, b.N, post2, s)) return rc;
    }
    return DPR_OK;
}

int njp_capture_graph(NjPruned& q, hipStream_t s, const std::function<int()>& enqueue)
{
    const auto t0 = std::chrono::steady_clock::now();
    ScopedGraph g;
    DPR_HIP(hipStreamBeginCapture(s, hipStreamCaptureModeThreadLocal));
    int rc = DPR_OK;
    for (int k = 0; k < q.graph_iters && rc == DPR_OK; ++k) rc = enqueue();
    hipError_t e = hipStreamEndCapture(s, g.put());
    if (rc != DPR_OK) return rc;
    if (e != hipSuccess) return hip_fail(e, "hipStreamEndCapture");
    e = hipGraphInstantiate(&q.graph, g, nullptr, nullptr, 0);
    if (e != hipSuccess) { q.graph = nullptr; return hip_fail(e, "hipGraphInstantiate"); }
    if (log_level("epoch") > 0)
        std::fprintf(stderr, "[njp] graph capture + instantiate (P=%lld): %.2f ms\n", (long long)q.P,
                     std::chrono::duration<double, std::milli>(std::chrono::steady_clock::now() - t0).count());
    return DPR_OK;
}

static int njp_run_segment(NjBuffers& b, int64_t it0, int64_t todo, hipStream_t s)
{
    NjPruned& q = b.pr;
    const int64_t limit = it0 + todo;
    DPR_HIP(hipMemcpyAsync(&b.st->it_limit, &limit, sizeof(int64_t), hipMemcpyHostToDevice, s));
    DPR_HIP(hipStreamSynchronize(s));
    if (todo <= 0) return DPR_OK;
    const int v0 = njp_first_rank(q), v1 = njp_last_rank(q);
    if (q.fresh) {
        for (int v = v0; v < v1; ++v)
            if (int rc = njp_launch_list_all(njp_args(b, v), s)) return rc;
        if (njp_use_post2(q)) {
            const int64_t S2 = (q.P + kTileCols - 1) / kTileCols + 2;
            const int par = (int)(it0 & 1);
            hipLaunchKernelGGL(njp_t2_init_kernel, dim3((unsigned)((q.P + kTileCols - 1) / kTileCols)), dim3(kThreads), 0, s,
                               (const double*)njp_current_u(q, it0), q.P, q.t2_rmax + par * 32 * S2, q.t2_cmax + par * 4 * S2);
            DPR_HIP(hipGetLastError());
        }
        q.fresh = false;
    }
    const bool timing = b.kt && b.kt->stride > 0 && q.sh_world <= 1;
    const bool use_graph = q.sh_world <= 1 && todo >= q.graph_iters && !timing;
    if (use_graph && !q.graph)
        if (int rc = njp_capture_graph(q, s, [&] { return njp_enqueue_iteration(b, s); })) return rc;
    int64_t done = 0;
    if (use_graph)
        for (; done + q.graph_iters <= todo; done += q.graph_iters) DPR_HIP(hipGraphLaunch(q.graph, s));
    for (; done < todo; ++done)
        if (int rc = njp_enqueue_iteration(b, s, timing && (it0 + done) % b.kt->stride == 0)) return rc;
    return njp_launch_finish(njp_args(b, v0), s);
}

static const char* const kNjpKernelNames[] = { "njp_scan_kernel", "njp_post_kernel", "(empty event pair)", "" };
static const char* const* g_kernel_names = kNjpKernelNames;
void njp_set_kernel_names(const char* const* names) { g_kernel_names = names ? names : kNjpKernelNames; }
const char* njp_kernel_name(int idx)
{
    if (idx < 0 || idx >= kNjKernelsMax) return "";
    for (int k = 0; k <= idx; ++k)
        if (g_kernel_names[k][0] == 0) return "";
    return g_kernel_names[idx];
}

int njp_debug_list(NjBuffers& b, int32_t* out, int64_t cap, int64_t* count, int64_t* P, double* ur, int64_t urcap)
{
    NjPruned& q = b.pr;
    if (!q.active || q.slots_mode || q.sh_world > 1) { set_error("njp_debug_list: no single-rank pruned epoch"); return DPR_ERR_STATE; }
    DPR_HIP(hipDeviceSynchronize());
    NjState st;
    DPR_HIP(hipMemcpy(&st, b.st, sizeof(NjState), hipMemcpyDeviceToHost));
    const int64_t cnt = (int64_t)st.cnt_list[st.it % 3];
    *count = cnt; *P = q.P;
    const int64_t take = cnt < cap ? cnt : cap;
    if (take > 0) DPR_HIP(hipMemcpy(out, q.list, sizeof(int32_t) * (size_t)take, hipMemcpyDeviceToHost));
    const int64_t tu = q.P < urcap ? q.P : urcap;
    if (ur && tu > 0) DPR_HIP(hipMemcpy(ur, q.Ur, sizeof(double) * (size_t)tu, hipMemcpyDeviceToHost));
    return DPR_OK;
}

int njp_phase_stamps(unsigned long long* out)
{
    if (!g_njp_dbg_last) { set_error("DPR_NJ_PHASES not set"); return DPR_ERR_STATE; }
    DPR_HIP(hipDeviceSynchronize());
    DPR_HIP(hipMemcpy(out, g_njp_dbg_last, sizeof(unsigned long long) * 4 * 2048 * 8, hipMemcpyDeviceToHost));
    return DPR_OK;
}

const double* njp_current_u(const NjPruned& q, int64_t it) { return q.U + (it & 1) * q.vstride; }

int njp_shape(const NjPruned& q, int64_t* positions, int* row_groups, int* strips, int* post2, int* scan_grid)
{
    if (positions) *positions = q.P;
    if (row_groups) *row_groups = njp_tg(q.P);
    if (strips) *strips = njp_ns(q.P);
    if (post2) *post2 = njp_use_post2(q) ? 1 : 0;
    if (scan_grid) *scan_grid = q.scan_grid;
    return DPR_OK;
}

constexpr int64_t kEpochPct = 80;
int64_t njp_epoch_min()
{
    const char* e = std::getenv("DPR_NJ_EPOCH_MIN");
    return e ? std::atoll(e) : 2048;
}
bool njp_epoch_due(int64_t P, int64_t n, int64_t left, int64_t epoch_min, int64_t* seg)
{
    *seg = left;
    if (epoch_min <= 0 || P < epoch_min) return false;
    const int64_t target = P * kEpochPct / 100;
    if (n <= target && n >= 3) return true;
    if (n - target < left) *seg = n - target;
    return false;
}

int njp_run(NjBuffers& b, int64_t it0, int64_t todo, hipStream_t s)
{
    const int64_t epoch_min = njp_epoch_min();
    NjPruned& q = b.pr;
    int64_t it = it0, left = todo;
    if (left <= 0) return q.slots_mode ? DPR_OK : njp_run_segment(b, it0, 0, s);
    while (left > 0) {
        const int64_t n = b.N - it;
        if (q.slots_mode) {
            if (n <= q.slots_probe_n && n >= epoch_min && n >= 3) {
                if (int rc = njp_from_slots(b, s)) return rc;
                if (!q.slots_mode) continue;
            }
            int64_t seg = left;
            if (n > q.slots_probe_n && q.slots_probe_n >= epoch_min && n - q.slots_probe_n < seg) seg = n - q.slots_probe_n;
            if (int rc = njp_run_slots(b, it, seg, s)) return rc;
            it += seg; left -= seg;
            continue;
        }
        int64_t seg = left;
        if (njp_epoch_due(q.P, n, left, epoch_min, &seg)) {
            DPR_HIP(hipStreamSynchronize(s));
            const auto t0 = std::chrono::steady_clock::now();
            bool rebuilt = false;
            if (int rc = njp_rebuild_epoch(b, s, &rebuilt)) return rc;
            if (!rebuilt) return DPR_OK;
            if (log_level("epoch") > 0)
                std::fprintf(stderr, "[njp] epoch rebuild at n=%lld: %.2f ms\n", (long long)n,
                             std::chrono::duration<double, std::milli>(std::chrono::steady_clock::now() - t0).count());
            continue;
        }
        const bool watch = q.adaptive && q.sh_world <= 1 && q.utot > 0;
        unsigned long long units0 = 0;
        bool first_of_epoch = false;
        if (watch) {
            first_of_epoch = q.fresh;
            const int64_t chunk = first_of_epoch ? (int64_t)q.graph_iters : 2048;
            if (seg > chunk) seg = chunk;
            NjState st0;
            DPR_HIP(hipStreamSynchronize(s));
            DPR_HIP(hipMemcpy(&st0, b.st, sizeof(NjState), hipMemcpyDeviceToHost));
            units0 = st0.units_scanned;
        }
        if (int rc = njp_run_segment(b, it, seg, s)) return rc;
        it += seg; left -= seg;
        if (watch && left > 0) {
            NjState st1;
            DPR_HIP(hipStreamSynchronize(s));
            DPR_HIP(hipMemcpy(&st1, b.st, sizeof(NjState), hipMemcpyDeviceToHost));
            if (st1.status != 0) continue;
            const double listed = (double)(st1.units_scanned - units0) - (first_of_epoch ? (double)q.utot : 0.0);
            const double iters = (double)seg - (first_of_epoch ? 1.0 : 0.0);
            const double rate = iters >= 1.0 ? listed / (iters * (double)q.utot) : 0.0;
            const double per_it = iters >= 1.0 ? listed / iters : 0.0;
            if (log_level("epoch") >= 2)
                std::fprintf(stderr, "[njp] watch at n=%lld: %.0f units per iteration over %.0f iterations (first of epoch %d, P=%lld, utot=%lld, scan grid %d)\n",
                             (long long)(b.N - it), per_it, iters, (int)first_of_epoch, (long long)q.P, (long long)q.utot, q.scan_grid);
            if (iters >= 1.0 && rate > q.stream_frac) {
                const int64_t na = b.N - it;
                int64_t pn = na;
                const int hops = 1 << (q.probe_fail_streak < 4 ? q.probe_fail_streak : 4);
                for (int h = 0; h < hops; ++h) pn = pn * kEpochPct / 100;
                ++q.probe_fail_streak;
                q.slots_probe_n = pn;
                if (int rc = njp_to_slots(b, s)) return rc;
                if (log_level("epoch") > 0)
                    std::fprintf(stderr, "[njp] %.0f %% of the units listed per iteration at n=%lld: handed over to the streaming loop; next pruned probe at n <= %lld\n",
                                 100.0 * rate, (long long)na, (long long)pn);
            } else if (!first_of_epoch) {
                q.probe_fail_streak = 0;
            }
        }
    }
    return DPR_OK;
}

}
```

### dipper_amd/csrc/njp_args.hpp

```cpp
#pragma once
#include "nj_dev.hpp"

#include <functional>

namespace dpr {

constexpr int kUR = 16;

__device__ __forceinline__ uint64_t enc_f64(double x)
{
    const uint64_t b = (uint64_t)__double_as_longlong(x);
    return (b >> 63) ? ~b : (b | 0x8000000000000000ull);
}
__device__ __forceinline__ double dec_f64(uint64_t k)
{
    const uint64_t b = (k >> 63) ? (k & 0x7fffffffffffffffull) : ~k;
    return __longlong_as_double((long long)b);
}
inline uint64_t enc_f64_host(double x)
{
    union { double d; uint64_t u; } c;
    c.d = x;
    return (c.u >> 63) ? ~c.u : (c.u | 0x8000000000000000ull);
}

__host__ __device__ inline int64_t unit_prefix(int64_t cb, int64_t G16) { return cb * G16 - 16 * cb * (cb - 1); }
__host__ __device__ inline int64_t unit_total(int64_t P)
{
    const int64_t G16 = (P + kUR - 1) / kUR;
    int64_t S = (P - 1 + kTileCols - 1) / kTileCols;
    while (S > 0 && G16 - 32 * (S - 1) <= 0) --S;
    return S > 0 ? unit_prefix(S, G16) : 0;
}



struct NjpArgs {
    double* D; int64_t ld; NjState* st;
    double* U; double* R; int64_t vstride;
    double* Ur; uint64_t* KA; uint64_t* KB; int32_t* slot_of_pos; int32_t* pos_of_slot;
    double* xpart; NjRecord* partials; unsigned long long* umin;
    int64_t P;
    const int32_t* blk_cb; const int32_t* blk_g0; int ntest;
    int tg, ns;
    int nupd;
    int32_t* list; unsigned long long* cnt;
    int ugrid;
    int urecs;
    int nrb;
    int rec_off;
    int all_defined;
    int sh_rank, sh_world;
    unsigned long long* cnt_all; int cnt_ranks;
    int do_update, do_tests, do_rows;
    int32_t* log_x; int32_t* log_y; double* log_bx; double* log_by;
    unsigned long long* dbg; int64_t dbg_it;
    void* t2_hdr; double* t2_rmax; double* t2_cmax; double* t2_colmin; double* t2_rowmin; double* t2_cmin;
    int rs_world, rs_rank;
    unsigned int rs_inv16;
    int64_t rs_slice;
    const double* rs_rows;
    int rs_plan;
    char* const* rs_win;
    NjrLayout rs_lay;
    unsigned int* rs_ticket;
    unsigned long long rs_seq_base, rs_poll_ticks;
    int64_t rs_fault_it;
};

template <bool kRS> __device__ __forceinline__ int64_t njp_lrow(const NjpArgs& a, int64_t p)
{
    if (!kRS) return p;
    const unsigned int k = (unsigned int)(p >> 10), kq = (k * a.rs_inv16) >> 16;
    return ((int64_t)kq << 10) | (p & 1023);
}
template <bool kRS> __device__ __forceinline__ bool njp_owns(const NjpArgs& a, int64_t p)
{
    if (!kRS) return true;
    const unsigned int k = (unsigned int)(p >> 10), kq = (k * a.rs_inv16) >> 16;
    return (int)(k - kq * (unsigned int)a.rs_world) == a.rs_rank;
}
__device__ __forceinline__ int64_t njp_xoff(const NjpArgs& a, int64_t p)
{
    const unsigned int k = (unsigned int)(p >> 10), kq = (k * a.rs_inv16) >> 16;
    const unsigned int o = k - kq * (unsigned int)a.rs_world;
    return (int64_t)(2u * o) * a.rs_slice + (((int64_t)kq << 10) | (p & 1023));
}

__device__ __forceinline__ void njr_st_sys(unsigned long long* p, unsigned long long v) { __hip_atomic_store(p, v, __ATOMIC_RELAXED, __HIP_MEMORY_SCOPE_SYSTEM); }
__device__ __forceinline__ unsigned long long njr_ld_sys(const unsigned long long* p) { return __hip_atomic_load(p, __ATOMIC_RELAXED, __HIP_MEMORY_SCOPE_SYSTEM); }
__device__ __forceinline__ void njr_st_flag(unsigned long long* p, unsigned long long v)
{
    asm volatile("s_waitcnt vmcnt(0)" ::: "memory");
    __hip_atomic_store(p, v, __ATOMIC_RELAXED, __HIP_MEMORY_SCOPE_SYSTEM);
}
__device__ __forceinline__ void njr_store_record(NjRecord* dst, double q, unsigned long long key, double d, unsigned long long pad)
{
    unsigned long long* w = reinterpret_cast<unsigned long long*>(dst);
    __hip_atomic_store(w + 0, (unsigned long long)__double_as_longlong(q), __ATOMIC_RELAXED, __HIP_MEMORY_SCOPE_AGENT);
    __hip_atomic_store(w + 1, key, __ATOMIC_RELAXED, __HIP_MEMORY_SCOPE_AGENT);
    __hip_atomic_store(w + 2, (unsigned long long)__double_as_longlong(d), __ATOMIC_RELAXED, __HIP_MEMORY_SCOPE_AGENT);
    __hip_atomic_store(w + 3, pad, __ATOMIC_RELAXED, __HIP_MEMORY_SCOPE_AGENT);
}
__device__ __forceinline__ char* njr_win_recs(char* region, const NjrLayout& lay, int parity, int src_rank)
{
    return region + lay.off_recs + (int64_t)sizeof(NjRecord) * ((int64_t)(parity * kNjsMaxWorld + src_rank) * lay.rec_stride);
}
__device__ __forceinline__ unsigned long long* njr_win_recflag(char* region, const NjrLayout& lay, int parity, int src_rank)
{
    return reinterpret_cast<unsigned long long*>(region + lay.off_recflag) + 8 * (parity * kNjsMaxWorld + src_rank);
}
__device__ __forceinline__ unsigned long long* njr_win_rowflag(char* region, const NjrLayout& lay, int src_rank)
{
    return reinterpret_cast<unsigned long long*>(region + lay.off_rowflag) + 8 * src_rank;
}
__device__ __forceinline__ bool njr_last_block(unsigned int* ticket, unsigned int* s_last)
{
    asm volatile("s_waitcnt vmcnt(0)" ::: "memory");
    __syncthreads();
    if (threadIdx.x == 0 && gridDim.x <= kNjsTicketGroups) {
        asm volatile("s_waitcnt vmcnt(0)" ::: "memory");
        const unsigned int tt = __hip_atomic_fetch_add(ticket, 1u, __ATOMIC_RELAXED, __HIP_MEMORY_SCOPE_AGENT);
        *s_last = (tt == gridDim.x - 1) ? 1u : 0u;
    } else if (threadIdx.x == 0) {
        asm volatile("s_waitcnt vmcnt(0)" ::: "memory");
        const unsigned int G = gridDim.x, grp = blockIdx.x % kNjsTicketGroups;
        const unsigned int in_grp = (G - grp + kNjsTicketGroups - 1) / kNjsTicketGroups, groups = G < kNjsTicketGroups ? G : kNjsTicketGroups;
        unsigned int last = 0u;
        const unsigned int t = __hip_atomic_fetch_add(ticket + 32 * (1 + grp), 1u, __ATOMIC_RELAXED, __HIP_MEMORY_SCOPE_AGENT);
        if (t == in_grp - 1) {
            const unsigned int tt = __hip_atomic_fetch_add(ticket, 1u, __ATOMIC_RELAXED, __HIP_MEMORY_SCOPE_AGENT);
            last = (tt == groups - 1) ? 1u : 0u;
        }
        *s_last = last;
    }
    __syncthreads();
    return *s_last != 0u;
}
__device__ __forceinline__ void njr_scan_publish(const NjpArgs& a, int64_t it, unsigned int* s_last)
{
    if (a.rs_plan != kNjrMailbox) return;
    if (!njr_last_block(a.rs_ticket, s_last)) return;
    const int tid = threadIdx.x;
    if (tid <= (int)kNjsTicketGroups) a.rs_ticket[32 * tid] = 0u;
    const int nrec = a.ugrid + 1, par = (int)(it & 1);
    const unsigned long long* src = reinterpret_cast<const unsigned long long*>(a.partials + a.rec_off - 1);
    const int words = 4 * nrec;
    for (int k0 = tid; k0 < words; k0 += 4 * kThreads) {
        unsigned long long v[4];
#pragma unroll
        for (int u = 0; u < 4; ++u) v[u] = (k0 + u * kThreads < words) ? __hip_atomic_load(src + k0 + u * kThreads, __ATOMIC_RELAXED, __HIP_MEMORY_SCOPE_AGENT) : 0ull;
        for (int peer = 0; peer < a.rs_world; ++peer) {
            unsigned long long* dst = reinterpret_cast<unsigned long long*>(njr_win_recs(a.rs_win[peer], a.rs_lay, par, a.rs_rank));
#pragma unroll
            for (int u = 0; u < 4; ++u)
                if (k0 + u * kThreads < words) njr_st_sys(dst + k0 + u * kThreads, v[u]);
        }
    }
    asm volatile("s_waitcnt vmcnt(0)" ::: "memory");
    __syncthreads();
    if (tid < a.rs_world) njr_st_flag(njr_win_recflag(a.rs_win[tid], a.rs_lay, par, a.rs_rank), a.rs_seq_base + (unsigned long long)(it + 1));
}

int njp_launch_list_all(const NjpArgs& a, hipStream_t s);
int njp_launch_scan(const NjpArgs& a, hipStream_t s);
int njp_launch_post(const NjpArgs& a, int64_t N, bool post2, hipStream_t s);
int njp_launch_finish(const NjpArgs& a, hipStream_t s);
int njp_rs_epoch(NjPruned& q, int64_t P, int64_t N, double* Dbuf, int epoch_index, int rs_rank, int rs_world, const void* hdr_from, hipStream_t s);
int njp_epoch_order(const double* dU, const int32_t* slot_of_pos, int64_t P, int64_t n, std::vector<int32_t>& perm, bool stream_idle, hipStream_t s);
int njp_init_vectors(NjPruned& q, const double* U_src, const int32_t* slot_src, int64_t n, int64_t it, hipStream_t s);
int njp_put_fresh_state(NjState* d_st, NjState& st, hipStream_t s);
void njp_plan_from_env(NjPruned& q);
int64_t njp_epoch_min();
bool njp_epoch_due(int64_t P, int64_t n, int64_t left, int64_t epoch_min, int64_t* seg);
int njp_capture_graph(NjPruned& q, hipStream_t s, const std::function<int()>& enqueue);

#define NJP_STAMP(k, j, drain)                                                                             \
    do {                                                                                                   \
        if (a.dbg != nullptr && it == a.dbg_it && threadIdx.x == 0) {                                      \
            if (drain) __builtin_amdgcn_s_waitcnt(0);                                                      \
            a.dbg[((k) * 2048 + (int)blockIdx.x) * 8 + (j)] = wall_clock64();                              \
        }                                                                                                  \
    } while (0)

__device__ __forceinline__ double nj_val(double dxi, double dyi, double d) { return (dxi + dyi - d) * 0.5; }
__device__ __forceinline__ double nj_unew(double up, double dxi, double dyi, double val) { return up + (-dxi - dyi + val); }

__device__ __forceinline__ void best_update4(double& bq, uint64_t& bk, uint64_t& bp, double& bd, double q, uint64_t k,
                                             uint64_t pp, double d)
{
    const bool take = (q < bq) | ((q == bq) & (k < bk));
    bq = take ? q : bq; bk = take ? k : bk; bp = take ? pp : bp; bd = take ? d : bd;
}


}
```

### dipper_amd/csrc/njr.hip

```cpp
#include "njp_args.hpp"

#include <algorithm>
#include <chrono>
#include <cstdio>
#include <cstdlib>

namespace dpr {

static size_t align256(size_t v) { return (v + 255) / 256 * 256; }

NjrLayout njr_layout(int64_t N, int world)
{
    NjrLayout l;
    l.rec_stride = 1024 / (world > 0 ? world : 1) + 1;
    l.slice = njr_slice_len(N, world);
    l.off_recflag = 0;
    l.off_recs = (int64_t)(2 * 64 * kNjsMaxWorld);
    l.off_rowflag = (int64_t)align256((size_t)l.off_recs + sizeof(NjRecord) * (size_t)(2 * kNjsMaxWorld) * (size_t)l.rec_stride);
    l.off_rows = l.off_rowflag + 64 * kNjsMaxWorld;
    l.bytes = l.off_rows + (int64_t)sizeof(double) * 2 * world * l.slice;
    return l;
}

static int64_t njr_local_count(int64_t P, int rank, int world)
{
    const int64_t full = P / kNjrChunk, rem = P % kNjrChunk;
    int64_t cnt = (full / world + ((full % world) > rank ? 1 : 0)) * kNjrChunk;
    if (rem && (full % world) == rank) cnt += rem;
    return cnt;
}

__global__ __launch_bounds__(kThreads) void njr_extract_kernel(NjpArgs a, int64_t rows_local)
{
    __shared__ double sq[kThreads / 64], sdd[kThreads / 64];
    __shared__ uint64_t sk[kThreads / 64], spp[kThreads / 64];
    __shared__ unsigned long long s_hdr[kNjsMaxWorld], s_seq[kNjsMaxWorld];
    __shared__ int s_fail;
    __shared__ unsigned int s_last;
    const int tid = threadIdx.x;
    const int64_t it = a.st->it, limit = a.st->it_limit, N = a.st->N;
    if (a.st->status != 0 || it >= limit) return;
    const int64_t n = N - it;
    if (n < 3) return;
    const int W = a.rs_world, rank = a.rs_rank, nrec = a.ugrid + 1, par = (int)(it & 1);
    const bool mailbox = a.rs_plan == kNjrMailbox;
    const unsigned long long want = a.rs_seq_base + (unsigned long long)(it + 1);
    if (tid == 0) s_fail = 0;
    __syncthreads();
    if (mailbox && tid < W) {
        const unsigned long long* f = njr_win_recflag(a.rs_win[rank], a.rs_lay, par, tid);
        const unsigned long long t0 = wall_clock64();
        while (njr_ld_sys(f) != want) {
            if (wall_clock64() - t0 > a.rs_poll_ticks) { s_fail = 3; break; }
            __builtin_amdgcn_s_sleep(1);
        }
    }
    __syncthreads();
    if (s_fail) {
        if (blockIdx.x == 0 && tid == 0) a.st->status = s_fail;
        return;
    }
    double bq = 10000.0, d = 0.0; uint64_t bk = ~0ull, bp = 0;
    constexpr int kPre = 4;
    for (int idx0 = tid; idx0 < W * nrec; idx0 += kPre * kThreads) {
        unsigned long long w4[kPre][4];
#pragma unroll
        for (int u = 0; u < kPre; ++u) {
            const int idx = idx0 + u * kThreads;
            w4[u][0] = (unsigned long long)__double_as_longlong(10000.0); w4[u][1] = ~0ull; w4[u][2] = 0ull; w4[u][3] = 0ull;
            if (idx >= W * nrec) continue;
            const int r = idx / nrec, k = idx - r * nrec;
            if (mailbox) {
                const unsigned long long* w = reinterpret_cast<const unsigned long long*>(njr_win_recs(a.rs_win[rank], a.rs_lay, par, r)) + 4 * k;
#pragma unroll
                for (int c = 0; c < 4; ++c) w4[u][c] = njr_ld_sys(w + c);
            } else {
                const unsigned long long* w = reinterpret_cast<const unsigned long long*>(a.partials + idx);
#pragma unroll
                for (int c = 0; c < 4; ++c) w4[u][c] = w[c];
            }
        }
#pragma unroll
        for (int u = 0; u < kPre; ++u) {
            const int idx = idx0 + u * kThreads;
            if (idx >= W * nrec) continue;
            const int r = idx / nrec, k = idx - r * nrec;
            const double q = __longlong_as_double((long long)w4[u][0]), dd = __longlong_as_double((long long)w4[u][2]);
            if (mailbox && blockIdx.x == 0) { NjRecord rec; rec.q = q; rec.key = w4[u][1]; rec.d = dd; rec.pad = w4[u][3]; a.partials[idx] = rec; }
            if (k == 0) { s_hdr[r] = w4[u][2]; s_seq[r] = w4[u][3]; }
            best_update4(bq, bk, bp, d, q, w4[u][1], w4[u][3], dd);
        }
    }
    for (int idx = tid; idx < a.nrb; idx += kThreads) {
        const NjRecord rec = a.partials[a.urecs + idx];
        best_update4(bq, bk, bp, d, rec.q, rec.key, rec.pad, rec.d);
    }
    wave_best4(bq, bk, bp, d);
    if ((tid & 63) == 0) { sq[tid >> 6] = bq; sk[tid >> 6] = bk; spp[tid >> 6] = bp; sdd[tid >> 6] = d; }
    __syncthreads();
    bq = sq[0]; bk = sk[0]; bp = spp[0]; d = sdd[0];
#pragma unroll
    for (int w = 1; w < kThreads / 64; ++w) best_update4(bq, bk, bp, d, sq[w], sk[w], spp[w], sdd[w]);
    if (tid < W) {
        if (s_seq[tid] != want) s_fail = 3;
        else if (s_hdr[tid] != s_hdr[rank]) s_fail = 4;
    }
    __syncthreads();
    if (s_fail) {
        if (blockIdx.x == 0 && tid == 0) {
            a.st->status = s_fail;
            if (s_fail == 4) {
                int other = 0;
                for (int r = 0; r < W; ++r) if (s_hdr[r] != s_hdr[rank]) { other = r; break; }
                a.st->q = __longlong_as_double((long long)s_hdr[rank]); a.st->d = __longlong_as_double((long long)s_hdr[other]);
                a.st->x = rank; a.st->y = other;
            }
        }
        return;
    }
    if (bk == ~0ull || !(bq < 10000.0)) return;
    const int64_t ki = (int64_t)(bk & 0xFFFFFFull), kj = (int64_t)((bk >> 24) & 0xFFFFFFull);
    const int64_t pi = (int64_t)(bp & 0xffffffffull), pj = (int64_t)(bp >> 32);
    const int64_t px = ki < kj ? pi : pj, py = ki < kj ? pj : pi;
    double* own_x = const_cast<double*>(a.rs_rows) + (int64_t)(2 * rank) * a.rs_slice;
    double* own_y = own_x + a.rs_slice;
    for (int64_t l = (int64_t)blockIdx.x * kThreads + tid; l < rows_local; l += (int64_t)gridDim.x * kThreads) {
        const double vx = a.D[l * a.ld + px], vy = a.D[l * a.ld + py];
        if (mailbox) {
            const unsigned long long ux = (unsigned long long)__double_as_longlong(vx), uy = (unsigned long long)__double_as_longlong(vy);
            for (int r = 0; r < W; ++r) {
                unsigned long long* dst = reinterpret_cast<unsigned long long*>(a.rs_win[r] + a.rs_lay.off_rows) + (int64_t)(2 * rank) * a.rs_slice + l;
                njr_st_sys(dst, ux);
                njr_st_sys(dst + a.rs_slice, uy);
            }
        } else {
            own_x[l] = vx; own_y[l] = vy;
        }
    }
    if (!mailbox) return;
    unsigned int* tk = a.rs_ticket + kNjsTicketBytes / sizeof(unsigned int);
    if (!njr_last_block(tk, &s_last)) return;
    if (tid <= (int)kNjsTicketGroups) tk[32 * tid] = 0u;
    if (tid < W) njr_st_flag(njr_win_rowflag(a.rs_win[tid], a.rs_lay, rank), want);
}

__global__ void njr_barrier_kernel(char* const* win, NjrLayout lay, int rank, int world, unsigned long long epoch, unsigned long long poll_ticks, NjState* st)
{
    const int tid = threadIdx.x;
    if (tid >= world) return;
    unsigned long long* theirs = njr_win_rowflag(win[tid], lay, rank) + 1;
    njr_st_flag(theirs, epoch);
    const unsigned long long* mine = njr_win_rowflag(win[rank], lay, tid) + 1;
    const unsigned long long t0 = wall_clock64();
    while (njr_ld_sys(mine) < epoch) {
        if (wall_clock64() - t0 > poll_ticks) { st->status = 3; break; }
        __builtin_amdgcn_s_sleep(4);
    }
}

__global__ __launch_bounds__(kThreads) void njr_stage_kernel(double* const* __restrict__ src, int64_t ld_src, int blk, int world, int64_t ncols,
                                                             const int32_t* __restrict__ perm, int64_t P, int64_t l0, int count, int rank,
                                                             double* __restrict__ stage, int64_t stage_ld)
{
    for (int i = blockIdx.y; i < count; i += gridDim.y) {
        const int64_t a = njr_global_pos(l0 + i, rank, world);
        if (a >= P) continue;
        const int64_t sr = perm[a], sb = sr / blk;
        const double* row = src[sb % world] + ((sb / world) * blk + sr % blk) * ld_src;
        double* dst = stage + (int64_t)i * stage_ld;
        for (int64_t c = ((int64_t)blockIdx.x * kThreads + threadIdx.x) * 2; c < ncols; c += (int64_t)gridDim.x * kThreads * 2) {
            const unsigned long long v0 = njr_ld_sys(reinterpret_cast<const unsigned long long*>(row + c));
            const unsigned long long v1 = njr_ld_sys(reinterpret_cast<const unsigned long long*>(row + c + 1));
            dst[c] = __longlong_as_double((long long)v0);
            dst[c + 1] = __longlong_as_double((long long)v1);
        }
    }
}
__global__ __launch_bounds__(kThreads) void njr_gather_kernel(const double* __restrict__ stage, int64_t stage_ld, const int32_t* __restrict__ perm, int64_t P,
                                                              double* __restrict__ B, int64_t ldb, int64_t l0, int count, int rank, int world)
{
    const int xcd = (int)(blockIdx.x & 7u), chunk = (int)(blockIdx.x >> 3), nchunk = (int)(gridDim.x >> 3);
    for (int i = (int)blockIdx.y * 8 + xcd; i < count; i += (int)gridDim.y * 8) {
        if (njr_global_pos(l0 + i, rank, world) >= P) continue;
        const double* row = stage + (int64_t)i * stage_ld;
        double* out = B + (l0 + i) * ldb;
        for (int64_t b = (int64_t)chunk * kThreads + threadIdx.x; b < P; b += (int64_t)nchunk * kThreads) out[b] = row[perm[b]];
    }
}

void njr_free(NjBuffers& b)
{
    NjRowShard& r = b.rs;
    void* ptrs[] = { r.rows_plain, r.stage, r.d_region, r.d_src, r.ticket };
    for (void* p : ptrs)
        if (p) (void)hipFree(p);
    NjRowShard fresh;
    fresh.gather = r.gather; fresh.barrier = r.barrier; fresh.cb_ctx = r.cb_ctx;
    r = fresh;
}

static NjpArgs njr_args(NjBuffers& b)
{
    NjPruned& q = b.pr;
    NjRowShard& r = b.rs;
    NjpArgs a{};
    a.D = q.D; a.ld = q.ld; a.st = b.st;
    a.U = q.U; a.R = q.R; a.vstride = q.vstride;
    a.Ur = q.Ur; a.KA = q.KA; a.KB = q.KB; a.slot_of_pos = q.slot_of_pos; a.pos_of_slot = q.pos_of_slot;
    a.xpart = b.xpart; a.partials = b.partials; a.umin = (unsigned long long*)q.umin;
    a.P = q.P;
    a.blk_cb = q.blk_cb; a.blk_g0 = q.blk_g0; a.ntest = q.nprep;
    a.tg = kNjrChunk / kUR; a.ns = 1; a.nupd = 0;
    a.list = q.list; a.cnt = b.st->cnt_list;
    a.ugrid = q.scan_grid / r.world > 0 ? q.scan_grid / r.world : 1;
    a.urecs = (a.ugrid + 1) * r.world;
    a.nrb = (int)((q.P + kTileCols - 1) / kTileCols);
    a.rec_off = r.rank * (a.ugrid + 1) + 1;
    a.all_defined = 1;
    a.sh_rank = 0; a.sh_world = 1;
    a.cnt_all = nullptr; a.cnt_ranks = 0;
    a.do_update = 1; a.do_tests = 1; a.do_rows = 1;
    a.log_x = b.log_x; a.log_y = b.log_y; a.log_bx = b.log_bx; a.log_by = b.log_by;
    a.dbg = nullptr; a.dbg_it = -1;
    a.t2_hdr = q.t2_hdr; a.t2_rmax = q.t2_rmax; a.t2_cmax = q.t2_cmax; a.t2_colmin = q.t2_colmin; a.t2_rowmin = q.t2_rowmin; a.t2_cmin = q.t2_cmin;
    a.rs_world = r.world; a.rs_rank = r.rank;
    a.rs_inv16 = (65536u + (unsigned int)r.world - 1u) / (unsigned int)r.world;
    a.rs_slice = r.lay.slice;
    a.rs_plan = r.plan;
    a.rs_lay = r.lay;
    a.rs_win = reinterpret_cast<char* const*>(r.d_region);
    a.rs_rows = r.plan == kNjrMailbox ? reinterpret_cast<const double*>(b.peer.win + r.win_off + r.lay.off_rows) : r.rows_plain;
    a.rs_ticket = r.ticket;
    a.rs_seq_base = b.peer.run_id << 32;
    a.rs_poll_ticks = b.peer.poll_ticks;
    a.rs_fault_it = b.peer.fault_rank == r.rank ? b.peer.fault_it : -1;
    return a;
}

static int njr_launch_extract(NjBuffers& b, hipStream_t s)
{
    const NjpArgs a = njr_args(b);
    const int64_t rows_local = njr_local_count(b.pr.P, b.rs.rank, b.rs.world);
    int64_t grid = (rows_local + kThreads - 1) / kThreads;
    grid = grid < 1 ? 1 : (grid > 32 ? 32 : grid);
    hipLaunchKernelGGL(njr_extract_kernel, dim3((unsigned)grid), dim3(kThreads), 0, s, a, rows_local);
    DPR_HIP(hipGetLastError());
    return DPR_OK;
}

static int njr_barrier(std::vector<NjBuffers*>& ranks, hipStream_t s)
{
    NjBuffers& b0 = *ranks[0];
    if (ranks.size() > 1) return DPR_OK;
    if (b0.rs.barrier) return b0.rs.barrier(b0.rs.cb_ctx);
    hipLaunchKernelGGL(njr_barrier_kernel, dim3(1), dim3(kNjsMaxWorld), 0, s, reinterpret_cast<char* const*>(b0.rs.d_region), b0.rs.lay, b0.rs.rank, b0.rs.world,
                       ++b0.peer.bar_epoch, b0.peer.poll_ticks, b0.st);
    DPR_HIP(hipGetLastError());
    DPR_HIP(hipStreamSynchronize(s));
    return DPR_OK;
}

static int njr_permute(NjBuffers& b, int src_half, int64_t ld_src, int blk, int64_t ncols, double* dst, int64_t ldb, int64_t P, hipStream_t s)
{
    NjRowShard& r = b.rs;
    const int64_t rows_local = njr_local_count(P, r.rank, r.world);
    double** d_src = r.d_src;
    DPR_HIP(hipMemcpyAsync(d_src, r.peer_half[src_half].data(), sizeof(double*) * (size_t)r.world, hipMemcpyHostToDevice, s));
    int64_t chunks = (P + 1023) / 1024;
    chunks = chunks < 1 ? 1 : (chunks > 64 ? 64 : chunks);
    for (int64_t l0 = 0; l0 < rows_local; l0 += r.stage_rows) {
        const int count = (int)(rows_local - l0 < r.stage_rows ? rows_local - l0 : r.stage_rows);
        int64_t gx = (ncols / 2 + kThreads - 1) / kThreads;
        gx = gx < 1 ? 1 : (gx > 64 ? 64 : gx);
        hipLaunchKernelGGL(njr_stage_kernel, dim3((unsigned)gx, (unsigned)count), dim3(kThreads), 0, s, (double* const*)d_src, ld_src, blk, r.world, ncols,
                           (const int32_t*)b.pr.perm, P, l0, count, r.rank, r.stage, r.stage_ld);
        hipLaunchKernelGGL(njr_gather_kernel, dim3((unsigned)(8 * chunks), (unsigned)((count + 7) / 8)), dim3(kThreads), 0, s, (const double*)r.stage, r.stage_ld,
                           (const int32_t*)b.pr.perm, P, dst, ldb, l0, count, r.rank, r.world);
    }
    DPR_HIP(hipGetLastError());
    DPR_HIP(hipStreamSynchronize(s));
    return DPR_OK;
}

static int njr_ensure_buffers(NjBuffers& b, hipStream_t s)
{
    NjRowShard& r = b.rs;
    if (b.twin_rows <= 0 || !b.D) { set_error("njr: the matrix buffers of this rank were not allocated for the row-sharded pruned plan"); return DPR_ERR_STATE; }
    r.lay = njr_layout(b.N, r.world);
    r.half[0] = b.D;
    r.half[1] = reinterpret_cast<double*>(reinterpret_cast<char*>(b.D) + b.half_bytes);
    if (r.plan == kNjrCollective && !r.rows_plain) {
        DPR_HIP(hipMalloc(&r.rows_plain, sizeof(double) * (size_t)(2 * r.world) * (size_t)r.lay.slice));
        DPR_HIP(hipMemsetAsync(r.rows_plain, 0, sizeof(double) * (size_t)(2 * r.world) * (size_t)r.lay.slice, s));
    }
    if (!r.d_region) {
        DPR_HIP(hipMalloc(&r.d_region, sizeof(char*) * kNjsMaxWorld));
        DPR_HIP(hipMalloc(&r.d_src, sizeof(double*) * kNjsMaxWorld));
        DPR_HIP(hipMalloc(&r.ticket, 2 * kNjsTicketBytes));
        DPR_HIP(hipMemsetAsync(r.ticket, 0, 2 * kNjsTicketBytes, s));
    }
    {
        if ((int)b.peer.h_D.size() != r.world || (r.plan == kNjrMailbox && (int)b.peer.h_win.size() != r.world)) {
            set_error("njr: the peers' buffers are not mapped on this rank"); return DPR_ERR_STATE;
        }
        std::vector<char*> regions((size_t)r.world, nullptr);
        for (int h = 0; h < 2; ++h) r.peer_half[h].assign((size_t)r.world, nullptr);
        for (int k = 0; k < r.world; ++k) {
            if ((int)b.peer.h_win.size() == r.world && b.peer.h_win[(size_t)k]) regions[(size_t)k] = b.peer.h_win[(size_t)k] + r.win_off;
            r.peer_half[0][(size_t)k] = b.peer.h_D[(size_t)k];
            r.peer_half[1][(size_t)k] = reinterpret_cast<double*>(reinterpret_cast<char*>(b.peer.h_D[(size_t)k]) + b.half_bytes);
        }
        DPR_HIP(hipMemcpyAsync(r.d_region, regions.data(), sizeof(char*) * (size_t)r.world, hipMemcpyHostToDevice, s));
        DPR_HIP(hipStreamSynchronize(s));
    }
    if (!r.stage) {
        r.stage_ld = (b.N + kTileCols + 16 + 15) / 16 * 16;
        int64_t rows = (int64_t)(256ll << 20) / (r.stage_ld * 8);
        rows = rows < 16 ? 16 : (rows > 1024 ? 1024 : rows);
        r.stage_rows = rows;
        DPR_HIP(hipMalloc(&r.stage, sizeof(double) * (size_t)(r.stage_rows * r.stage_ld)));
    }
    return DPR_OK;
}

int njr_build(std::vector<NjBuffers*>& ranks, hipStream_t s)
{
    NjBuffers& b0 = *ranks[0];
    const int64_t N = b0.N;
    std::vector<int32_t> perm;
    if (int rc = njp_epoch_order(b0.U, nullptr, N, N, perm, false, s)) return rc;
    for (NjBuffers* pb : ranks) {
        NjBuffers& b = *pb;
        if (int rc = njr_ensure_buffers(b, s)) return rc;
        njp_plan_from_env(b.pr);
        DPR_HIP(hipMemsetAsync(b.rs.half[1], 0, b.half_bytes, s));
        if (int rc = njp_rs_epoch(b.pr, N, N, b.rs.half[1], 0, b.rs.rank, b.rs.world, nullptr, s)) return rc;
        b.pr.utot0 = b.pr.utot;
        DPR_HIP(hipMemcpyAsync(b.pr.perm, perm.data(), sizeof(int32_t) * (size_t)N, hipMemcpyHostToDevice, s));
    }
    if (int rc = njr_barrier(ranks, s)) return rc;
    for (NjBuffers* pb : ranks) {
        NjBuffers& b = *pb;
        if (int rc = njr_permute(b, 0, b.ld, kRowBlock, N, b.pr.D, b.pr.ld, N, s)) return rc;
        if (int rc = njp_init_vectors(b.pr, b.U, nullptr, N, 0, s)) return rc;
    }
    DPR_HIP(hipStreamSynchronize(s));
    return njr_barrier(ranks, s);
}

static int njr_rebuild_epoch(std::vector<NjBuffers*>& ranks, hipStream_t s, bool* rebuilt)
{
    NjBuffers& b0 = *ranks[0];
    *rebuilt = false;
    NjState st;
    DPR_HIP(hipMemcpy(&st, b0.st, sizeof(NjState), hipMemcpyDeviceToHost));
    const int64_t n = st.n, Pold = b0.pr.P;
    if (st.status != 0 || n < 3) return DPR_OK;
    std::vector<int32_t> perm;
    if (int rc = njp_epoch_order(njp_current_u(b0.pr, st.it), b0.pr.slot_of_pos, Pold, n, perm, true, s)) return rc;
    if (int rc = njr_barrier(ranks, s)) return rc;
    const int e = b0.pr.epoch_index + 1;
    const int src_half = (b0.pr.epoch_index + 1) & 1, dst_half = (e + 1) & 1;
    for (NjBuffers* pb : ranks) {
        NjBuffers& b = *pb;
        const NjPruned old = b.pr;
        DPR_HIP(hipMemsetAsync(b.rs.half[dst_half], 0, b.half_bytes, s));
        if (int rc = njp_rs_epoch(b.pr, n, b.N, b.rs.half[dst_half], e, b.rs.rank, b.rs.world, nullptr, s)) return rc;
        DPR_HIP(hipMemcpyAsync(b.pr.perm, perm.data(), sizeof(int32_t) * (size_t)n, hipMemcpyHostToDevice, s));
        if (int rc = njr_permute(b, src_half, old.ld, kNjrChunk, Pold, b.pr.D, b.pr.ld, n, s)) return rc;
        if (int rc = njp_init_vectors(b.pr, njp_current_u(old, st.it), old.slot_of_pos, n, st.it, s)) return rc;
        if (int rc = njp_put_fresh_state(b.st, st, s)) return rc;
        DPR_HIP(hipStreamSynchronize(s));
    }
    if (int rc = njr_barrier(ranks, s)) return rc;
    *rebuilt = true;
    return DPR_OK;
}

static const char* const kNjrKernelNames[] = { "njp_scan_kernel<rs>", "(other ranks' launches / exchange)", "njr_extract_kernel", "(other ranks' launches / exchange)",
                                               "njp_post_kernel<64,1,rs>", "" };
static int njr_iteration(std::vector<NjBuffers*>& ranks, hipStream_t s, bool sample)
{
    NjBuffers& b0 = *ranks[0];
    NjKernelTiming* kt = b0.kt;
    if (sample) { kt->nk = 5; njp_set_kernel_names(kNjrKernelNames); }
    for (size_t r = 0; r < ranks.size(); ++r) {
        if (int rc = nj_timing_mark(kt, sample && r == 0, s)) return rc;
        if (int rc = njp_launch_scan(njr_args(*ranks[r]), s)) return rc;
        if (int rc = nj_timing_mark(kt, sample && r == 0, s)) return rc;
    }
    if (b0.rs.plan == kNjrCollective) { if (int rc = b0.rs.gather(b0.rs.cb_ctx, 0, s)) return rc; ++b0.rs.collectives; }
    for (size_t r = 0; r < ranks.size(); ++r) {
        if (int rc = nj_timing_mark(kt, sample && r == 0, s)) return rc;
        if (int rc = njr_launch_extract(*ranks[r], s)) return rc;
        if (int rc = nj_timing_mark(kt, sample && r == 0, s)) return rc;
    }
    if (b0.rs.plan == kNjrCollective) { if (int rc = b0.rs.gather(b0.rs.cb_ctx, 1, s)) return rc; ++b0.rs.collectives; }
    for (size_t r = 0; r < ranks.size(); ++r) {
        if (int rc = nj_timing_mark(kt, sample && r == 0, s)) return rc;
        if (int rc = njp_launch_post(njr_args(*ranks[r]), ranks[r]->N, false, s)) return rc;
        if (int rc = nj_timing_mark(kt, sample && r == 0, s)) return rc;
    }
    b0.rs.launches += 3;
    return DPR_OK;
}

static int njr_run_segment(std::vector<NjBuffers*>& ranks, int64_t it0, int64_t todo, hipStream_t s)
{
    const int64_t limit = it0 + todo;
    for (NjBuffers* pb : ranks) DPR_HIP(hipMemcpyAsync(&pb->st->it_limit, &limit, sizeof(int64_t), hipMemcpyHostToDevice, s));
    DPR_HIP(hipStreamSynchronize(s));
    if (todo <= 0) return DPR_OK;
    for (NjBuffers* pb : ranks) {
        if (!pb->pr.fresh) continue;
        if (int rc = njp_launch_list_all(njr_args(*pb), s)) return rc;
        pb->pr.fresh = false;
    }
    NjBuffers& b0 = *ranks[0];
    const bool timing = b0.kt && b0.kt->stride > 0;
    const int gi = b0.pr.graph_iters;
    const bool use_graph = ranks.size() == 1 && b0.rs.plan == kNjrMailbox && todo >= gi && !timing;
    if (use_graph && !b0.pr.graph) {
        if (int rc = njp_capture_graph(b0.pr, s, [&] { return njr_iteration(ranks, s, false); })) return rc;
        b0.rs.launches -= 3 * gi;
    }
    int64_t done = 0;
    if (use_graph)
        for (; done + gi <= todo; done += gi) { DPR_HIP(hipGraphLaunch(b0.pr.graph, s)); b0.rs.launches += 3 * gi; }
    for (; done < todo; ++done)
        if (int rc = njr_iteration(ranks, s, timing && (it0 + done) % b0.kt->stride == 0)) return rc;
    for (NjBuffers* pb : ranks)
        if (int rc = njp_launch_finish(njr_args(*pb), s)) return rc;
    return DPR_OK;
}

int njr_run(std::vector<NjBuffers*>& ranks, int64_t it0, int64_t todo, hipStream_t s)
{
    const int64_t epoch_min = njp_epoch_min();
    NjBuffers& b0 = *ranks[0];
    int64_t it = it0, left = todo;
    if (left <= 0) return njr_run_segment(ranks, it0, 0, s);
    while (left > 0) {
        int64_t seg = left;
        if (njp_epoch_due(b0.pr.P, b0.N - it, left, epoch_min, &seg)) {
            DPR_HIP(hipStreamSynchronize(s));
            bool rebuilt = false;
            if (int rc = njr_rebuild_epoch(ranks, s, &rebuilt)) return rc;
            if (!rebuilt) return DPR_OK;
            continue;
        }
        if (int rc = njr_run_segment(ranks, it, seg, s)) return rc;
        it += seg; left -= seg;
    }
    return njr_barrier(ranks, s);
}

}
```

Baseline: 33540.

## Split each NJ scan unit across two blocks by row halves

In the non-row-sharded path, each listed scan unit (kUR rows by one column tile) is now processed by two blocks, each handling half the rows. The grid and the partial-record count double, and the umin array gets two slots per wave. Post kernels take the min of the two halves and scan both seed records per entry. The aim is to cut tail latency from long-running unit blocks by giving each block less work, at the cost of more blocks, more records to reduce and a larger umin footprint.

```diff
diff --git a/dipper_amd/csrc/njp.hip b/dipper_amd/csrc/njp.hip
--- a/dipper_amd/csrc/njp.hip
+++ b/dipper_amd/csrc/njp.hip
@@ -156,7 +156,7 @@
     }
 }
 
-template <bool kRS>
+template <bool kRS, int kH>
 __global__ __launch_bounds__(kThreads) void njp_scan_kernel(NjState* h_st, const int32_t* h_list, const unsigned long long* h_cnt,
                                                             const double* h_xpart, int h_nrl, NjpArgs a)
 {
@@ -170,7 +170,9 @@
     const int nrl = h_nrl;
     const bool unit_block = (int)blockIdx.x >= nrl;
     const int ub = (int)blockIdx.x - nrl;
-    const int32_t first = unit_block ? h_list[ub] : 0;
+    constexpr int kR = kUR / kH;
+    const int ue = ub / kH, uh = ub - ue * kH;
+    const int32_t first = unit_block ? h_list[ue] : 0;
     const double xp0 = unit_block ? 0.0 : h_xpart[tid];
     const unsigned long long cl0 = h_cnt[0], cl1 = h_cnt[1], cl2 = h_cnt[2];
     const int64_t j0 = (int64_t)blockIdx.x * kTileCols + 2 * tid;
@@ -233,7 +235,7 @@
         rec_out = a.partials + a.rec_off + ub;
         const int m3 = (int)(it % 3);
         const int64_t cnt = (int64_t)(m3 == 0 ? cl0 : m3 == 1 ? cl1 : cl2);
-        if ((int64_t)ub >= cnt) {
+        if ((int64_t)ue >= cnt) {
             if (a.all_defined && tid == 0) {
                 if (kRS) njr_store_record(rec_out, 10000.0, ~0ull, 0.0, 0ull);
                 else { NjRecord rec; rec.q = 10000.0; rec.key = ~0ull; rec.d = 0.0; rec.pad = 0ull; *rec_out = rec; }
@@ -244,12 +246,12 @@
         const int64_t G16 = (P + kUR - 1) / kUR;
         int64_t scanned = 0;
         const int wv = tid >> 6;
-        for (int64_t e = ub; e < cnt; e += a.ugrid, ++scanned) {
-            const uint32_t code = (uint32_t)__builtin_amdgcn_readfirstlane(e == (int64_t)ub ? first : a.list[e]);
+        for (int64_t e = ue; e < cnt; e += a.ugrid, ++scanned) {
+            const uint32_t code = (uint32_t)__builtin_amdgcn_readfirstlane(e == (int64_t)ue ? first : a.list[e]);
             if (!((code >> (28 + wv)) & 1u)) continue;
             const int cb = (int)((code >> 18) & 1023u);
             const int64_t g_s = (int64_t)(code & 0x3FFFFu);
-            const int64_t c0 = (int64_t)cb * kTileCols, a0 = g_s * kUR;
+            const int64_t c0 = (int64_t)cb * kTileCols, a0 = g_s * kUR + uh * kR;
             const int64_t b0 = c0 + 2 * tid, b1 = b0 + 1;
             const v2d ubv = *reinterpret_cast<const v2d*>(a.Ur + b0);
             const ulonglong2 kav = *reinterpret_cast<const ulonglong2*>(a.KA + b0), kbv = *reinterpret_cast<const ulonglong2*>(a.KB + b0);
@@ -259,28 +261,28 @@
             const int64_t ld2 = a.ld >> 1;
             const bool diag = a0 < c0 + kTileCols;
             const bool live0 = ub0 == ub0, live1 = ub1 == ub1;
-            v2d v[kUR];
-#pragma unroll
-            for (int u8 = 0; u8 < kUR; ++u8) v[u8] = __builtin_nontemporal_load(basep + (int64_t)u8 * ld2);
-            const double ua_l = a.Ur[a0 + (tid & 15)];
-            const uint64_t kaa_l = a.KA[a0 + (tid & 15)], kba_l = a.KB[a0 + (tid & 15)];
-            double ua[kUR];
-#pragma unroll
-            for (int u8 = 0; u8 < kUR; ++u8) ua[u8] = readlane_f64(ua_l, u8);
+            v2d v[kR];
+#pragma unroll
+            for (int u8 = 0; u8 < kR; ++u8) v[u8] = __builtin_nontemporal_load(basep + (int64_t)u8 * ld2);
+            const double ua_l = a.Ur[a0 + (tid & (kR - 1))];
+            const uint64_t kaa_l = a.KA[a0 + (tid & (kR - 1))], kba_l = a.KB[a0 + (tid & (kR - 1))];
+            double ua[kR];
+#pragma unroll
+            for (int u8 = 0; u8 < kR; ++u8) ua[u8] = readlane_f64(ua_l, u8);
             NJP_STAMP(0, 1, true);
             if (diag) {
                 const int ib0 = (int)b0, ia0 = (int)a0;
 #pragma unroll
-                for (int u8 = 0; u8 < kUR; ++u8) {
+                for (int u8 = 0; u8 < kR; ++u8) {
                     const int ar = ia0 + u8;
                     v[u8].x = (ib0 < ar) ? v[u8].x : __builtin_nan("");
                     v[u8].y = (ib0 + 1 < ar) ? v[u8].y : __builtin_nan("");
                 }
             }
             double lm = __builtin_inf(), m0 = __builtin_inf(), m1 = __builtin_inf();
-            double rowq[kUR];
-#pragma unroll
-            for (int u8 = 0; u8 < kUR; ++u8) {
+            double rowq[kR];
+#pragma unroll
+            for (int u8 = 0; u8 < kR; ++u8) {
                 const double d0 = v[u8].x, d1 = v[u8].y;
                 const double rn = ua[u8] == ua[u8] ? 0.0 : __builtin_nan("");
                 m0 = fmin(m0, d0 + rn);
@@ -299,7 +301,7 @@
                 if (wm < bq) { bq = wm; bk = ~0ull; }
                 if (a.dbg != nullptr && (it == a.dbg_it || a.dbg_it == -2) && (tid & 63) == 0) atomicAdd(&a.dbg[(a.dbg_it == -2 ? 0 : (int)blockIdx.x) * 8 + 6], 1ull);
 #pragma unroll
-                for (int u8 = 0; u8 < kUR; ++u8) {
+                for (int u8 = 0; u8 < kR; ++u8) {
                     if (__builtin_amdgcn_ballot_w64(rowq[u8] == wm) != 0ull) {
                         if (a.dbg != nullptr && (it == a.dbg_it || a.dbg_it == -2) && (tid & 63) == 0) atomicAdd(&a.dbg[(a.dbg_it == -2 ? 0 : (int)blockIdx.x) * 8 + 5], 1ull);
                         double d0 = v[u8].x, d1 = v[u8].y;
@@ -318,7 +320,11 @@
             }
             NJP_STAMP(0, 7, false);
             m = wave_fmin(m);
-            if ((tid & 63) == 0) a.umin[((int64_t)cb * G16 + g_s) * 4 + wv] = enc_f64(m);
+            if ((tid & 63) == 0) {
+                unsigned long long* um = a.umin + (((int64_t)cb * G16 + g_s) * 4 + wv) * 2;
+                if (kH == 1) *reinterpret_cast<ulonglong2*>(um) = make_ulonglong2(enc_f64(m), enc_f64(__builtin_inf()));
+                else um[uh] = enc_f64(m);
+            }
         }
         {
             const uint64_t wk = wave_umin64(bk);
@@ -402,16 +408,21 @@
     }
     const int nseed_rows = a.nrb < kThreads / 2 ? a.nrb : kThreads / 2;
     const int nseed_units = kThreads - nseed_rows;
-    const int64_t sstride = a.all_defined && a.urecs >= 2 * nseed_units ? a.urecs / nseed_units : 1;
+    const int nent = a.urecs / a.halves;
+    const int64_t sstride = a.all_defined && nent >= 2 * nseed_units ? nent / nseed_units : 1;
     const bool seed_is_unit = tid < nseed_units;
-    NjRecord cand = r0;
+    const int64_t seed_rec = (int64_t)tid * sstride * a.halves;
+    NjRecord cand = r0, cand2 = r0;
     if (test_block) {
         if (!seed_is_unit) cand = h_partials[a.urecs + (tid - nseed_units)];
-        else if ((int64_t)tid * sstride < a.urecs) cand = h_partials[(int64_t)tid * sstride];
+        else if (seed_rec < a.urecs) {
+            cand = h_partials[seed_rec];
+            if (a.halves == 2) cand2 = h_partials[seed_rec + 1];
+        }
     }
     const unsigned long long cl0 = h_cnt[0], cl1 = h_cnt[1], cl2 = h_cnt[2];
     const int m3 = (int)(it % 3);
-    const unsigned long long cnt_raw = a.all_defined ? (unsigned long long)a.urecs : (m3 == 0 ? cl0 : m3 == 1 ? cl1 : cl2);
+    const unsigned long long cnt_raw = a.all_defined ? (unsigned long long)a.urecs : (unsigned long long)a.halves * (m3 == 0 ? cl0 : m3 == 1 ? cl1 : cl2);
     const int64_t uvalid = (int64_t)(cnt_raw < (unsigned long long)a.urecs ? cnt_raw : (unsigned long long)a.urecs);
     const double* __restrict__ Uc = a.U + (it & 1) * a.vstride;
     double* __restrict__ Un = a.U + ((it + 1) & 1) * a.vstride;
@@ -421,7 +432,7 @@
     const int64_t i = (int64_t)ubi * kThreads + tid;
     int64_t p = -1;
     double up = 0.0;
-    struct ColData { v2d ucol, dxc, dyc, rzc; ulonglong2 um0, um1; };
+    struct ColData { v2d ucol, dxc, dyc, rzc; ulonglong2 um[4]; };
     int cb0 = 0, nsb = 0;
     int64_t g = 0, rbase = 0;
     bool have_g = false;
@@ -431,14 +442,16 @@
 #pragma unroll
     for (int k = 0; k < kNS; ++k) {
         cd[k].ucol.x = 0.0; cd[k].ucol.y = 0.0; cd[k].dxc = cd[k].ucol; cd[k].dyc = cd[k].ucol; cd[k].rzc = cd[k].ucol;
-        cd[k].um0 = make_ulonglong2(0ull, 0ull); cd[k].um1 = cd[k].um0;
+#pragma unroll
+        for (int w = 0; w < 4; ++w) cd[k].um[w] = make_ulonglong2(0ull, 0ull);
     }
     auto load_a = [&](int cb, ColData& c) {
         const int64_t pc0 = (int64_t)cb * kTileCols + 2 * tid;
         c.ucol = *reinterpret_cast<const v2d*>(Uc + pc0);
         if (have_g && g >= 32 * (int64_t)cb) {
-            const unsigned long long* up = a.umin + ((int64_t)cb * G16 + g) * 4;
-            c.um0 = *reinterpret_cast<const ulonglong2*>(up); c.um1 = *reinterpret_cast<const ulonglong2*>(up + 2);
+            const ulonglong2* up = reinterpret_cast<const ulonglong2*>(a.umin + ((int64_t)cb * G16 + g) * 8);
+#pragma unroll
+            for (int w = 0; w < 4; ++w) c.um[w] = up[w];
         }
     };
     if (test_block) {
@@ -608,7 +621,8 @@
     for (int k = 0; k < kNS; ++k)
         if (k < nsb) load_b(cb0 + k, cd[k]);
     double qc = PINF;
-    if (seed_is_unit && (int64_t)tid * sstride >= uvalid) cand.key = ~0ull;
+    if (seed_is_unit && seed_rec >= uvalid) { cand.key = ~0ull; cand2.key = ~0ull; }
+    if (cand2.key != ~0ull && (cand.key == ~0ull || cand2.q < cand.q)) cand = cand2;
     if (cand.key != ~0ull) {
         const int64_t ci = (int64_t)(cand.pad & 0xffffffffull), cj = (int64_t)(cand.pad >> 32);
         if (ci < P && cj < P && ci != px && cj != px && ci != py && cj != py) {
@@ -649,9 +663,12 @@
         const int64_t pc0 = (int64_t)cb * kTileCols + 2 * tid;
         const bool pz_strip = fold && pz / kTileCols == cb;
         const bool have = have_g && g >= 32 * (int64_t)cb;
-        unsigned long long* up4 = a.umin + ((int64_t)cb * G16 + (have ? g : 0)) * 4;
+        ulonglong2* up4 = reinterpret_cast<ulonglong2*>(a.umin + ((int64_t)cb * G16 + (have ? g : 0)) * 8);
         double u4[4] = { PINF, PINF, PINF, PINF };
-        if (have) { u4[0] = dec_f64(cur.um0.x); u4[1] = dec_f64(cur.um0.y); u4[2] = dec_f64(cur.um1.x); u4[3] = dec_f64(cur.um1.y); }
+        if (have) {
+#pragma unroll
+            for (int w = 0; w < 4; ++w) u4[w] = dec_f64(cur.um[w].x < cur.um[w].y ? cur.um[w].x : cur.um[w].y);
+        }
         double cm_part = NINF, colmin = PINF;
 #pragma unroll
         for (int k = 0; k < 2; ++k) {
@@ -703,7 +720,7 @@
                 if (pz_strip && w == wpz) nm = fmin(nm, newminA);
                 if (nm < u4[w]) {
                     u4[w] = nm;
-                    up4[w] = enc_f64(nm);
+                    up4[w] = make_ulonglong2(enc_f64(nm), enc_f64(nm));
                 }
                 const double lb = fmin((u4[w] - rmax) - cmw, (u4[w] - cmw) - rmax);
                 if ((cmw > NINF) && (lb <= bound)) submask |= 1 << w;
@@ -780,9 +797,11 @@
     }
     const int nseed_rows = a.nrb < kThreads / 2 ? a.nrb : kThreads / 2;
     const int nseed_units = kThreads - nseed_rows;
-    const int64_t sstride = a.all_defined && a.urecs >= 2 * nseed_units ? a.urecs / nseed_units : 1;
+    const int nent = a.urecs / a.halves;
+    const int64_t sstride = a.all_defined && nent >= 2 * nseed_units ? nent / nseed_units : 1;
     const bool seed_is_unit = tid < nseed_units;
-    NjRecord cand = r0;
+    const int64_t seed_rec = (int64_t)tid * sstride * a.halves;
+    NjRecord cand = r0, cand2 = r0;
     int cb0 = 0;
     int64_t g0 = 0;
     const int64_t i = (int64_t)umb * (2 * kThreads) + tid;
@@ -793,7 +812,10 @@
     int2 sl = make_int2(-1, -1);
     if (trole) {
         if (!seed_is_unit) cand = h_partials[a.urecs + (tid - nseed_units)];
-        else if ((int64_t)tid * sstride < a.urecs) cand = h_partials[(int64_t)tid * sstride];
+        else if (seed_rec < a.urecs) {
+            cand = h_partials[seed_rec];
+            if (a.halves == 2) cand2 = h_partials[seed_rec + 1];
+        }
         cb0 = h_blk_cb[tb];
         g0 = (int64_t)h_blk_g0[tb];
     } else {
@@ -805,7 +827,7 @@
     double* __restrict__ Un = a.U + ((it + 1) & 1) * a.vstride;
     const unsigned long long cl0 = h_cnt[0], cl1 = h_cnt[1], cl2 = h_cnt[2];
     const int m3 = (int)(it % 3);
-    const unsigned long long cnt_raw = a.all_defined ? (unsigned long long)a.urecs : (m3 == 0 ? cl0 : m3 == 1 ? cl1 : cl2);
+    const unsigned long long cnt_raw = a.all_defined ? (unsigned long long)a.urecs : (unsigned long long)a.halves * (m3 == 0 ? cl0 : m3 == 1 ? cl1 : cl2);
     const int64_t uvalid = (int64_t)(cnt_raw < (unsigned long long)a.urecs ? cnt_raw : (unsigned long long)a.urecs);
     const double emin = dec_f64(hdr->min_enc), eabs = dec_f64(hdr->maxabs_enc);
     v2d uc; uc.x = 0.0; uc.y = 0.0;
@@ -820,7 +842,8 @@
         const int64_t send = njp_strips_of_rows(g0, kTG, P);
         nsb = (int)(send - cb0 < kNS ? send - cb0 : kNS);
         if (pz >= 0) uz = Uc[pz];
-        if (seed_is_unit && (int64_t)tid * sstride >= uvalid) cand.key = ~0ull;
+        if (seed_is_unit && seed_rec >= uvalid) { cand.key = ~0ull; cand2.key = ~0ull; }
+        if (cand2.key != ~0ull && (cand.key == ~0ull || cand2.q < cand.q)) cand = cand2;
         if (cand.key != ~0ull) {
             ci = (int64_t)(cand.pad & 0xffffffffull); cj = (int64_t)(cand.pad >> 32);
             if (!(ci < P && cj < P)) ci = -1;
@@ -1011,12 +1034,15 @@
         }
     }
     ulonglong2 um0[kNS], um1[kNS];
+    auto load_um = [&](int k) {
+        const ulonglong2* up = reinterpret_cast<const ulonglong2*>(a.umin + ((int64_t)(cb0 + k) * G16 + g) * 8);
+        const ulonglong2 p0 = up[0], p1 = up[1], p2 = up[2], p3 = up[3];
+        um0[k] = make_ulonglong2(p0.x < p0.y ? p0.x : p0.y, p1.x < p1.y ? p1.x : p1.y);
+        um1[k] = make_ulonglong2(p2.x < p2.y ? p2.x : p2.y, p3.x < p3.y ? p3.x : p3.y);
+    };
 #pragma unroll
     for (int k = 0; k < kNS; ++k) { um0[k] = make_ulonglong2(0ull, 0ull); um1[k] = um0[k]; }
-    if (kNS == 1 && nsb > 0 && have_g && g >= 32 * (int64_t)cb0) {
-        const unsigned long long* up = a.umin + ((int64_t)cb0 * G16 + g) * 4;
-        um0[0] = *reinterpret_cast<const ulonglong2*>(up); um1[0] = *reinterpret_cast<const ulonglong2*>(up + 2);
-    }
+    if (kNS == 1 && nsb > 0 && have_g && g >= 32 * (int64_t)cb0) load_um(0);
     qc = wave_fmin(qc);
     if (lane == 0) sseed[tid >> 6] = qc;
     NJP_STAMP(1, 3, true);
@@ -1067,10 +1093,7 @@
     if (kNS > 1) {
 #pragma unroll
         for (int k = 0; k < kNS; ++k) {
-            if (k < nsb && have_g && g >= 32 * (int64_t)(cb0 + k)) {
-                const unsigned long long* up = a.umin + ((int64_t)(cb0 + k) * G16 + g) * 4;
-                um0[k] = *reinterpret_cast<const ulonglong2*>(up); um1[k] = *reinterpret_cast<const ulonglong2*>(up + 2);
-            }
+            if (k < nsb && have_g && g >= 32 * (int64_t)(cb0 + k)) load_um(k);
         }
     }
     NJP_STAMP(1, 5, true);
@@ -1087,7 +1110,7 @@
         const int cb = cb0 + sidx;
         const bool pz_strip = fold && cbz == cb;
         const bool have = have_g && g >= 32 * (int64_t)cb;
-        unsigned long long* up4 = a.umin + ((int64_t)cb * G16 + (have ? g : 0)) * 4;
+        ulonglong2* up4 = reinterpret_cast<ulonglong2*>(a.umin + ((int64_t)cb * G16 + (have ? g : 0)) * 8);
         double u4[4] = { PINF, PINF, PINF, PINF };
         if (have) { u4[0] = dec_f64(um0[sidx].x); u4[1] = dec_f64(um0[sidx].y); u4[2] = dec_f64(um1[sidx].x); u4[3] = dec_f64(um1[sidx].y); }
         const double newminA = (pz_strip && have_g) ? a.t2_rowmin[par * GS + g] : PINF;
@@ -1100,7 +1123,7 @@
                 if (pz_strip && w == wpz) nm = fmin(nm, newminA);
                 if (nm < u4[w]) {
                     u4[w] = nm;
-                    up4[w] = enc_f64(nm);
+                    up4[w] = make_ulonglong2(enc_f64(nm), enc_f64(nm));
                 }
                 mymin = fmin(mymin, u4[w]);
                 const double lb = fmin((u4[w] - rmax) - cmw, (u4[w] - cmw) - rmax);
@@ -1144,8 +1167,8 @@
 static unsigned long long* g_njp_dbg_last = nullptr;
 
 [[maybe_unused]] static const void* const kNjpInstantiations[] = {
-    (const void*)njp_scan_kernel<false>, (const void*)njp_post2_kernel<kBigNS>, (const void*)njp_post_kernel<64, 1, false>, (const void*)njp_post_kernel<256, kBigNS, false>,
-    (const void*)njp_scan_kernel<true>, (const void*)njp_post_kernel<64, 1, true>, (const void*)njp_finish_kernel<true>, (const void*)njp_finish_kernel<false> };
+    (const void*)njp_scan_kernel<false, 2>, (const void*)njp_post2_kernel<kBigNS>, (const void*)njp_post_kernel<64, 1, false>, (const void*)njp_post_kernel<256, kBigNS, false>,
+    (const void*)njp_scan_kernel<true, 1>, (const void*)njp_post_kernel<64, 1, true>, (const void*)njp_finish_kernel<true>, (const void*)njp_finish_kernel<false> };
 
 int njp_launch_list_all(const NjpArgs& a, hipStream_t s)
 {
@@ -1156,8 +1179,9 @@
 int njp_launch_scan(const NjpArgs& a, hipStream_t s)
 {
     const int nrl = a.do_rows ? a.nrb : 0;
-    auto* kernel = a.rs_world > 0 ? njp_scan_kernel<true> : njp_scan_kernel<false>;
-    hipLaunchKernelGGL(kernel, dim3((unsigned)(a.ugrid + nrl)), dim3(kThreads), 0, s, a.st, (const int32_t*)a.list, (const unsigned long long*)a.cnt,
+    auto* kernel = a.rs_world > 0 ? njp_scan_kernel<true, 1> : njp_scan_kernel<false, 2>;
+    if (a.halves != (a.rs_world > 0 ? 1 : 2)) { set_error("njp_launch_scan: record layout does not match the kernel"); return DPR_ERR_STATE; }
+    hipLaunchKernelGGL(kernel, dim3((unsigned)(a.halves * a.ugrid + nrl)), dim3(kThreads), 0, s, a.st, (const int32_t*)a.list, (const unsigned long long*)a.cnt,
                        (const double*)a.xpart, nrl, a);
     DPR_HIP(hipGetLastError());
     return DPR_OK;
@@ -1241,7 +1265,7 @@
     take(q.slot_of_pos, vec, 0xff);
     take(q.pos_of_slot, vec, 0xff);
     take(q.perm, vec);
-    q.nunits_alloc = S * G16 * 4;
+    q.nunits_alloc = S * G16 * 8;
     take(q.umin, (size_t)q.nunits_alloc);
     q.list_stride = unit_total(P) + kScanBlocks + 64;
     take(q.list, (size_t)(q.list_stride * local_ranks), 0);
@@ -1537,6 +1561,7 @@
     q = NjPruned();
 }
 
+constexpr int kNjpHalves = 2;
 static int njp_grid_rank(const NjPruned& q) { return q.sh_world > 1 ? (q.scan_grid / q.sh_world > 0 ? q.scan_grid / q.sh_world : 1) : q.scan_grid; }
 static int njp_grid_total(const NjPruned& q) { return q.sh_world > 1 ? njp_grid_rank(q) * q.sh_world : q.scan_grid; }
 static int njp_first_rank(const NjPruned& q) { return q.sh_world > 1 && !q.sh_virtual ? q.sh_rank : 0; }
@@ -1559,9 +1584,10 @@
     a.list = q.list + (int64_t)slot * q.list_stride;
     a.cnt = sh ? q.cnt_all + 4 * slot : b.st->cnt_list;
     a.ugrid = njp_grid_rank(q);
-    a.urecs = njp_grid_total(q);
+    a.halves = kNjpHalves;
+    a.urecs = kNjpHalves * njp_grid_total(q);
     a.nrb = (int)((q.P + kTileCols - 1) / kTileCols);
-    a.rec_off = sh ? v * a.ugrid : 0;
+    a.rec_off = sh ? v * kNjpHalves * a.ugrid : 0;
     a.all_defined = sh ? 1 : 0;
     a.sh_rank = sh ? v : 0; a.sh_world = sh ? q.sh_world : 1;
     a.cnt_all = sh ? q.cnt_all : nullptr;
@@ -1595,7 +1621,7 @@
     }
     if (!q.sh_virtual) {
         if (!q.gather) { set_error("njp: unit-sharded mode without a gather callback"); return DPR_ERR_STATE; }
-        if (int rc = q.gather(q.gather_ctx, b.partials, sizeof(NjRecord) * (size_t)njp_grid_rank(q), s)) return rc;
+        if (int rc = q.gather(q.gather_ctx, b.partials, sizeof(NjRecord) * (size_t)(kNjpHalves * njp_grid_rank(q)), s)) return rc;
     }
     for (int v = v0; v < v1; ++v) {
         NjpArgs a = njp_args(b, v);
diff --git a/dipper_amd/csrc/njp_args.hpp b/dipper_amd/csrc/njp_args.hpp
--- a/dipper_amd/csrc/njp_args.hpp
+++ b/dipper_amd/csrc/njp_args.hpp
@@ -46,6 +46,7 @@
     int nupd;
     int32_t* list; unsigned long long* cnt;
     int ugrid;
+    int halves;
     int urecs;
     int nrb;
     int rec_off;
diff --git a/dipper_amd/csrc/njr.hip b/dipper_amd/csrc/njr.hip
--- a/dipper_amd/csrc/njr.hip
+++ b/dipper_amd/csrc/njr.hip
@@ -213,6 +213,7 @@
     a.tg = kNjrChunk / kUR; a.ns = 1; a.nupd = 0;
     a.list = q.list; a.cnt = b.st->cnt_list;
     a.ugrid = q.scan_grid / r.world > 0 ? q.scan_grid / r.world : 1;
+    a.halves = 1;
     a.urecs = (a.ugrid + 1) * r.world;
     a.nrb = (int)((q.P + kTileCols - 1) / kTileCols);
     a.rec_off = r.rank * (a.ugrid + 1) + 1;
diff --git a/profiles/nj_scan_tail.py b/profiles/nj_scan_tail.py
--- /dev/null
+++ b/profiles/nj_scan_tail.py
@@ -0,0 +1,82 @@
+import argparse, ctypes as C, json, os, subprocess, sys, tempfile
+
+ROOT = os.path.dirname(os.path.dirname(os.path.abspath(__file__)))
+sys.path.insert(0, ROOT)
+ap = argparse.ArgumentParser()
+ap.add_argument("--tips", type=int, default=30000)
+ap.add_argument("--sites", type=int, default=10000)
+ap.add_argument("--its", default="3000,12000,24000")
+ap.add_argument("--halves", type=int, default=1)
+ap.add_argument("--json", default=None)
+args = ap.parse_args()
+import torch
+import numpy as np
+import dipper_amd
+from dipper_amd import capi
+
+
+def alignment(n, L, seed=1):
+    tmp = tempfile.mkdtemp(prefix="njt_", dir="/dev/shm" if os.path.isdir("/dev/shm") else None)
+    p4 = os.path.join(tmp, "a.p4")
+    k = 10000.0 / L
+    subprocess.run([os.path.join(ROOT, "tools", "bin", "gen_synth"), "--tips", str(n), "--sites", str(L), "--seed", str(seed),
+                    "--mean-bl", repr(2e-5 * k), "--lo", repr(2e-6 * k), "--hi", repr(2e-4 * k), "--packed4", p4], check=True)
+    packed = np.fromfile(p4, dtype=np.uint64).reshape(n, (L + 15) // 16)
+    os.unlink(p4); os.rmdir(tmp)
+    return packed
+
+
+def positions_at(N, it, epoch_min=2048):
+    P = N
+    for i in range(it + 1):
+        n = N - i
+        if P >= epoch_min and n <= P * 80 // 100 and n >= 3:
+            P = n
+    return P
+
+
+packed = alignment(args.tips, args.sites)
+L_ = capi.load_library()
+L_.dpr_get_nj_phase_stamps.argtypes = [C.c_void_p]
+out = []
+for it in [int(x) for x in args.its.split(",")] + [-2]:
+    os.environ["DPR_NJ_PHASES"] = str(it)
+    d = dipper_amd.Dipper(0)
+    d.set_msa(packed, args.sites)
+    d.dist_matrix(capi.SRC_MSA, capi.DIST_JC)
+    d.nj_run()
+    nj_ms = d.timing()[1]
+    units = d.prune_stats()[0]
+    buf = np.zeros(4 * 2048 * 8, np.uint64)
+    assert L_.dpr_get_nj_phase_stamps(buf.ctypes.data) == 0
+    d.close()
+    if it == -2:
+        rec = {"iteration": -2, "nj_ms": nj_ms, "units_listed": int(units), "pass2_row_hits": int(buf[5]), "pass2_wave_unit_entries": int(buf[6]),
+               "hits_per_iteration": float(buf[5]) / (args.tips - 2), "entries_per_iteration": float(buf[6]) / (args.tips - 2)}
+        out.append(rec); print(json.dumps(rec), flush=True)
+        continue
+    b = buf[:2048 * 8].reshape(2048, 8).astype(np.int64)
+    used = b[:, 0] > 0
+    t0 = b[used][:, 0].min()
+    P = positions_at(args.tips, it)
+    nrb = (P + 511) // 512
+    idx = np.arange(2048)
+    done = used & (b[:, 4] > 0)
+    rec = {"iteration": it, "nj_ms": nj_ms, "positions": P, "new_row_blocks": nrb, "blocks_stamped": int(used.sum()), "blocks_with_work": int(done.sum())}
+    end = 10 * (b[:, 4] - t0)
+    for name, m in (("unit", done & (idx >= nrb)), ("new_row", done & (idx < nrb))):
+        if not m.any():
+            continue
+        e = end[m]
+        rec[name] = {"blocks": int(m.sum()), "median_end_ns": int(np.median(e)), "p90_end_ns": int(np.percentile(e, 90)), "slowest_end_ns": int(e.max()),
+                     "median_start_ns": int(np.median(10 * (b[m][:, 0] - t0))), "tied_rows_median": float(np.median(b[m][:, 5])), "tied_rows_max": int(b[m][:, 5].max())}
+    s = int(np.argmax(np.where(done, end, -1)))
+    rec["slowest_block"] = {"index": s, "role": "unit" if s >= nrb else "new_row", "end_ns": int(end[s]), "start_ns": int(10 * (b[s, 0] - t0)),
+                            "tied_rows": int(b[s, 5]) if s >= nrb else 0, "list_entry": (s - nrb) // args.halves if s >= nrb else -1}
+    order = [int(i) for i in np.argsort(np.where(done & (idx >= nrb), end, -1))[-8:][::-1]]
+    rec["slowest_unit_blocks"] = [{"end_ns": int(end[i]), "start_ns": int(10 * (b[i, 0] - t0)), "tied_rows": int(b[i, 5])} for i in order]
+    out.append(rec); print(json.dumps(rec), flush=True)
+if args.json:
+    os.makedirs(os.path.dirname(os.path.abspath(args.json)), exist_ok=True)
+    with open(args.json, "w") as f:
+        json.dump(out, f, indent=1)
```

New measurement: 34890 (median of 6 runs). 4.0% higher.
